# fanxiaochen/Multi-View-Registration

Hardware: NVIDIA B200
Metric: nn_queries_per_s (24-view x 200k turntable registration; ms_per_step = registration ms; a query = one PCL-equivalent nearest-neighbour answer: every source point per iteration + every gated match's reciprocal answer, the oracle's counter) (higher is better)
Workload: dtype f32

## Files before the change

### include/mvr_b200.h

```cpp
#ifndef MVR_B200_H
#define MVR_B200_H

#include <stddef.h>
#include <stdint.h>

#ifdef __cplusplus
extern "C" {
#endif

typedef struct mvr_ctx mvr_ctx;

typedef enum {
  MVR_OK = 0,
  MVR_ERR_BAD_ARG = 1,
  MVR_ERR_TOO_FEW_CORRESPONDENCES = 2,
  MVR_ERR_CUDA = 3,
  MVR_ERR_NO_INPUT = 4,
  MVR_ERR_NOT_SPD = 5,
  MVR_ERR_ALLOC = 6,
  MVR_ERR_NCCL = 7
} mvr_status;

typedef enum { MVR_CLOUD_TARGET = 0, MVR_CLOUD_SOURCE = 1 } mvr_cloud;
typedef enum { MVR_POINT_TO_POINT = 0, MVR_POINT_TO_PLANE = 1, MVR_SYMMETRIC = 2 } mvr_estimator;
typedef enum {
  MVR_REASON_NONE = 0,
  MVR_REASON_ITERATIONS = 1,
  MVR_REASON_TRANSFORM = 2,
  MVR_REASON_ABS_MSE = 3,
  MVR_REASON_REL_MSE = 4,
  MVR_REASON_NO_CORRESPONDENCES = 5
} mvr_reason;

typedef struct {
  int max_iterations;
  double max_correspondence_distance;
  double transformation_epsilon;
  double euclidean_fitness_epsilon;
  int use_reciprocal_correspondences;
  int estimator;
  int fixed_iterations;
  int min_correspondences;
} mvr_icp_params;

typedef struct {
  int iterations;
  int converged;
  int reason;
  int n_correspondences;
  double mse;
  double gpu_ms;
  uint64_t nn_queries;
} mvr_icp_report;

typedef struct {
  int iteration;
  int n_correspondences;
  double mse;
  float delta[16];
} mvr_icp_iteration;

typedef struct {
  float origin[3];
  float inv_cell;
  float cell;
  int bits;
} mvr_grid;

typedef struct {
  uint64_t launches;
  double ms;
  double bytes;
  double units;
} mvr_kernel_stat;

enum { MVR_K_MORTON = 0, MVR_K_SORT = 1, MVR_K_TABLE = 2, MVR_K_NN = 3, MVR_K_CORR = 4, MVR_K_REDUCE = 5,
       MVR_K_TRANSFORM = 6, MVR_K_NORMALS = 7, MVR_K_COUNT = 8 };

const char* mvr_version(void);
uint64_t mvr_kernel_launch_count(void);
void mvr_transfer_sizes(size_t* state_bytes, size_t* log_record_bytes);
const char* mvr_status_string(int status);
void mvr_icp_params_default(mvr_icp_params* p);

int mvr_ctx_create(int device, mvr_ctx** out);
int mvr_ctx_destroy(mvr_ctx* ctx);
int mvr_ctx_set_stream(mvr_ctx* ctx, void* cuda_stream);
int mvr_ctx_synchronize(mvr_ctx* ctx);
void* mvr_ctx_get_stream(mvr_ctx* ctx);
const char* mvr_last_error(mvr_ctx* ctx);
int mvr_ctx_set_profiling(mvr_ctx* ctx, int on);
int mvr_ctx_get_kernel_stats(mvr_ctx* ctx, mvr_kernel_stat* out , int reset);
double mvr_debug_value(mvr_ctx* ctx, int k);
int mvr_ctx_set_index_options(mvr_ctx* ctx, float cell_edge, int max_bits);

int mvr_ctx_set_nn_options(mvr_ctx* ctx, double points_per_cell, double dense_ratio);
typedef enum { MVR_NN_AUTO = 0, MVR_NN_WARP = 1, MVR_NN_THREAD = 2, MVR_NN_CELL = 3, MVR_NN_SEEDED = 4 } mvr_nn_mode;
int mvr_ctx_set_nn_mode(mvr_ctx* ctx, int mode);
int mvr_ctx_set_gate_mask(mvr_ctx* ctx, int on);

int mvr_set_target(mvr_ctx* ctx, const float* xyzw, size_t n);
int mvr_set_source(mvr_ctx* ctx, const float* xyzw, size_t n);
int mvr_set_target_device(mvr_ctx* ctx, const float* d_xyzw, size_t n);
int mvr_set_source_device(mvr_ctx* ctx, const float* d_xyzw, size_t n);
int mvr_set_clouds_device(mvr_ctx* const* ctxs, const int* which, const float* const* d_xyzw, const size_t* n, int count);
int mvr_cloud_share(mvr_ctx* dst, int which_dst , mvr_ctx* src, int which_src);
int mvr_set_target_normals(mvr_ctx* ctx, const float* nxyzc, size_t n);
int mvr_set_source_normals(mvr_ctx* ctx, const float* nxyzc, size_t n);
int mvr_normals_share(mvr_ctx* dst, int which_dst , mvr_ctx* src, int which_src);

int mvr_index_build(mvr_ctx* ctx, int which , const mvr_grid* grid );
int mvr_index_export(mvr_ctx* ctx, int which, mvr_grid* grid, uint32_t* sorted_keys, int32_t* perm,
                     uint32_t* cell_start);

int mvr_nn_query(mvr_ctx* ctx, const float* q_xyzw, size_t n, int32_t* idx, float* d2);
int mvr_nn_query_device(mvr_ctx* ctx, const float* d_q_xyzw, size_t n, int32_t* d_idx, float* d_d2);

int mvr_correspondences(mvr_ctx* ctx, double max_dist, int reciprocal, int32_t* index_query, int32_t* index_match,
                        float* distance, size_t* count);

int mvr_icp_align(mvr_ctx* ctx, const mvr_icp_params* params, const float* guess, float* out_pose, float* out_xyzw,
                  mvr_icp_report* report);
int mvr_icp_align_batch(mvr_ctx* const* ctxs, int count, const mvr_icp_params* params, const float* guesses, float* out_poses,
                        mvr_icp_report* reports, int* statuses);
int mvr_ctx_set_batch_group(mvr_ctx* ctx, int pairs);
int mvr_icp_get_iterations(mvr_ctx* ctx, mvr_icp_iteration* out, int max_records, int* count);
int mvr_fitness_score(mvr_ctx* ctx, double max_range, double* score);

typedef struct {
  double n;
  double origin[3];
  double sa[3], sb[3];
  double sba[9];
  double saa[6], sbb[6];
  double d2;
} mvr_pair_moments;
int mvr_pair_moments_compute(mvr_ctx* ctx, double max_dist, int reciprocal, const float* guess, mvr_pair_moments* out);

int mvr_pair_moments_compute_batch(mvr_ctx* const* ctxs, int count, double max_dist, int reciprocal, const float* guesses,
                                   mvr_pair_moments* out, int* statuses);

int mvr_estimate_normals(mvr_ctx* ctx, int which, int k, const float viewpoint[3], float* out_nxyzc,
                         int32_t* neighbours);
int mvr_estimate_normals_batch(mvr_ctx* const* ctxs, int count, int k, const float* viewpoints, float* const* out_nxyzc,
                               int* statuses);

int mvr_apply_pose(mvr_ctx* ctx, const void* points, size_t n, size_t stride_bytes, const double* pose, float* out_xyzw);
int mvr_apply_pose_device(mvr_ctx* ctx, const void* d_points, size_t n, size_t stride_bytes, const double* pose, float* d_out_xyzw);
int mvr_copy_aligned_device(mvr_ctx* ctx, float* d_out_xyzw);

typedef struct mvr_registrator mvr_registrator;

typedef struct {
  const float* xyzw;
  size_t n;
  int on_device;
  const double* init_pose;
} mvr_view;

typedef enum {
  MVR_REGISTER_RING_PAIRS = 0,
  MVR_REGISTER_ACCUMULATE = 1,
  MVR_REGISTER_ICP = 2,
  MVR_REGISTER_LUM = 3
} mvr_register_mode;

typedef struct {
  double pivot[3];
  double axis[3];
  mvr_icp_params icp;
  int repeat_times;
  int mode;
  int loop_closure;
  int lum_iterations;
  int pair_begin, pair_end;
  int want_fitness;
  int normal_k;
} mvr_turntable_params;

typedef struct {
  int source_view, target_view;
  int status;
  int iterations;
  int n_correspondences;
  double mse;
  double fitness;
  double gpu_ms;
  uint64_t nn_queries;
  float pose[16];
} mvr_pair_report;

typedef struct { int view; int repeat; double score; } mvr_fitness_record;

void mvr_turntable_params_default(mvr_turntable_params* p);
void mvr_turntable_rotation(const double pivot[3], const double axis[3], double angle, double* out16);
double mvr_turntable_view_angle(int view, int n_views);

int mvr_registrator_create(int device, int streams, mvr_registrator** out);
int mvr_registrator_destroy(mvr_registrator* r);
const char* mvr_registrator_last_error(mvr_registrator* r);
mvr_ctx* mvr_registrator_context(mvr_registrator* r, int slot);
int mvr_registrator_streams(mvr_registrator* r);
int mvr_pairwise_align(mvr_registrator* r, const mvr_view* source, const mvr_view* target, const mvr_icp_params* icp,
                       const float* guess, float* out_pose, mvr_icp_report* report);
int mvr_register_turntable(mvr_registrator* r, const mvr_view* views, int n_views, const mvr_turntable_params* prm,
                           float* poses, mvr_pair_report* reports);
typedef struct mvr_multi mvr_multi;
typedef struct {
  float pose[16];
  int32_t n_correspondences, iterations, status, reserved;
  double mse;
  uint64_t nn_queries;
} mvr_pair_record;
int mvr_multi_create(const int* devices, int n_devices, mvr_multi** out);
int mvr_multi_destroy(mvr_multi* m);
const char* mvr_multi_last_error(mvr_multi* m);
int mvr_multi_devices(mvr_multi* m);
int mvr_multi_contexts(mvr_multi* m, int rank);
mvr_ctx* mvr_multi_context(mvr_multi* m, int rank, int slot);
void mvr_multi_pair_range(int rank, int n_ranks, int n_pairs, int* pair_begin, int* pair_end);
int mvr_multi_upload(mvr_multi* m, const mvr_view* views, int n_views);
int mvr_register_turntable_multi(mvr_multi* m, const mvr_view* views, int n_views, const mvr_turntable_params* prm, int use_resident,
                                 float* poses, mvr_pair_report* reports, mvr_pair_record* records, double* device_ms);

int mvr_registrator_get_fitness_log(mvr_registrator* r, mvr_fitness_record* out, int max_records, int* count);
int mvr_compute_error(mvr_registrator* r, const mvr_view* views, int n_views, double max_distance, size_t* counts, double* mean_d2,
                      int* n_pairs);
int mvr_ring_close(const float* rel_poses, const double* weights, int n_views, int relax, int iterations, const double* centre,
                   double rot_scale, float* poses);
int mvr_lum_relax(const mvr_pair_moments* edges, const int* src, const int* tgt, int n_edges, int n_views, int iterations,
                  double* poses);
int mvr_lum_compute(const mvr_pair_moments* edges, const int* src, const int* tgt, int n_edges, int n_views, int iterations,
                    double convergence_threshold, double* poses6, double* transforms);
void mvr_pair_moments_transform(const mvr_pair_moments* in, const double* pose, const double* new_origin, mvr_pair_moments* out);
int mvr_get_bbox(mvr_ctx* ctx, int which, float lo[3], float hi[3]);
int mvr_refine_axis(const float* poses, int count, double pivot[3], double axis[3]);

int mvr_transformation_load(const char* path, double* pose);
int mvr_transformation_save(const char* path, const double* pose);
int mvr_axis_load(const char* path, double pivot[3], double axis[3]);
int mvr_axis_save(const char* path, const double pivot[3], const double axis[3]);
int mvr_points_save_asc(const char* path, const void* rich_points, size_t n);
int mvr_merge_registered(mvr_ctx* ctx, const void* const* views, const size_t* counts, const double* poses, const int* registered,
                         int n_views, int full_matrix_normals, void* out, size_t* out_count);

int mvr_denoise(mvr_ctx* ctx, const void* points, size_t n, size_t stride_bytes, int segment_threshold, double triangle_length,
// ... 7 lines not shown
```

### multi-view-registration_b200/__init__.py

```python
import ctypes as C
import os

import numpy as np

_HERE = os.path.dirname(os.path.abspath(__file__))
LIB_PATH = os.environ.get("MVR_B200_LIB") or os.path.join(_HERE, "libmvr_b200.so")

K_NAMES = ["morton", "sort", "table", "nn", "corr", "reduce", "transform", "normals"]
K_COUNT = 8
(OK, ERR_BAD_ARG, ERR_TOO_FEW, ERR_CUDA, ERR_NO_INPUT, ERR_NOT_SPD, ERR_ALLOC, ERR_NCCL) = range(8)
TARGET, SOURCE = 0, 1
NN_AUTO, NN_WARP, NN_THREAD, NN_CELL, NN_SEEDED = 0, 1, 2, 3, 4
POINT_TO_POINT, POINT_TO_PLANE, SYMMETRIC = 0, 1, 2


class MvrError(RuntimeError):
    def __init__(self, status, msg):
        super().__init__("mvr status %d: %s" % (status, msg))
        self.status = status


class IcpParams(C.Structure):
    _fields_ = [
        ("max_iterations", C.c_int),
        ("max_correspondence_distance", C.c_double),
        ("transformation_epsilon", C.c_double),
        ("euclidean_fitness_epsilon", C.c_double),
        ("use_reciprocal_correspondences", C.c_int),
        ("estimator", C.c_int),
        ("fixed_iterations", C.c_int),
        ("min_correspondences", C.c_int),
    ]


class IcpReport(C.Structure):
    _fields_ = [
        ("iterations", C.c_int),
        ("converged", C.c_int),
        ("reason", C.c_int),
        ("n_correspondences", C.c_int),
        ("mse", C.c_double),
        ("gpu_ms", C.c_double),
        ("nn_queries", C.c_uint64),
    ]


class IcpIteration(C.Structure):
    _fields_ = [("iteration", C.c_int), ("n_correspondences", C.c_int), ("mse", C.c_double), ("delta", C.c_float * 16)]


class Grid(C.Structure):
    _fields_ = [("origin", C.c_float * 3), ("inv_cell", C.c_float), ("cell", C.c_float), ("bits", C.c_int)]


class KernelStat(C.Structure):
    _fields_ = [("launches", C.c_uint64), ("ms", C.c_double), ("bytes", C.c_double), ("units", C.c_double)]


class TurntableParams(C.Structure):
    _fields_ = [
        ("pivot", C.c_double * 3),
        ("axis", C.c_double * 3),
        ("icp", IcpParams),
        ("repeat_times", C.c_int),
        ("mode", C.c_int),
        ("loop_closure", C.c_int),
        ("lum_iterations", C.c_int),
        ("pair_begin", C.c_int),
        ("pair_end", C.c_int),
        ("want_fitness", C.c_int),
        ("normal_k", C.c_int),
    ]


class PairMoments(C.Structure):
    _fields_ = [("n", C.c_double), ("origin", C.c_double * 3), ("sa", C.c_double * 3), ("sb", C.c_double * 3),
                ("sba", C.c_double * 9), ("saa", C.c_double * 6), ("sbb", C.c_double * 6), ("d2", C.c_double)]

    @classmethod
    def from_pairs(cls, a, b, origin=None):
        a = np.asarray(a, dtype=np.float64).reshape(-1, 3)
        b = np.asarray(b, dtype=np.float64).reshape(-1, 3)
        o = np.zeros(3) if origin is None else np.asarray(origin, dtype=np.float64)
        m = cls()
        m.n = float(len(a))
        m.origin[:] = o.tolist()
        if len(a):
            x, y = a - o, b - o
            m.sa[:] = x.sum(0).tolist(); m.sb[:] = y.sum(0).tolist()
            m.sba[:] = (y.T @ x).reshape(9).tolist()
            xx, yy = x.T @ x, y.T @ y
            m.saa[:] = [xx[0, 0], xx[0, 1], xx[0, 2], xx[1, 1], xx[1, 2], xx[2, 2]]
            m.sbb[:] = [yy[0, 0], yy[0, 1], yy[0, 2], yy[1, 1], yy[1, 2], yy[2, 2]]
            m.d2 = float(((a - b) ** 2).sum())
        return m

    def as_dict(self):
        return dict(n=self.n, origin=np.array(self.origin[:]), sa=np.array(self.sa[:]), sb=np.array(self.sb[:]),
                    sba=np.array(self.sba[:]).reshape(3, 3), saa=np.array(self.saa[:]), sbb=np.array(self.sbb[:]), d2=self.d2)


class ViewDesc(C.Structure):
    _fields_ = [("xyzw", C.c_void_p), ("n", C.c_size_t), ("on_device", C.c_int), ("init_pose", C.POINTER(C.c_double))]


class PairRecord(C.Structure):
    _fields_ = [("pose", C.c_float * 16), ("n_correspondences", C.c_int32), ("iterations", C.c_int32), ("status", C.c_int32),
                ("reserved", C.c_int32), ("mse", C.c_double), ("nn_queries", C.c_uint64)]


class FitnessRecord(C.Structure):
    _fields_ = [("view", C.c_int), ("repeat", C.c_int), ("score", C.c_double)]


class PairReport(C.Structure):
    _fields_ = [
        ("source_view", C.c_int),
        ("target_view", C.c_int),
        ("status", C.c_int),
        ("iterations", C.c_int),
        ("n_correspondences", C.c_int),
        ("mse", C.c_double),
        ("fitness", C.c_double),
        ("gpu_ms", C.c_double),
        ("nn_queries", C.c_uint64),
        ("pose", C.c_float * 16),
    ]


REPORT = np.dtype([("source_view", "<i4"), ("target_view", "<i4"), ("status", "<i4"), ("iterations", "<i4"), ("n_correspondences", "<i4"),
                   ("pad", "<i4"), ("mse", "<f8"), ("fitness", "<f8"), ("gpu_ms", "<f8"), ("nn_queries", "<u8"), ("pose", "<f4", (16,))])
assert REPORT.itemsize == C.sizeof(PairReport)


class BoundViews:

    def __init__(self, arr, keep, n, views):
        self.arr, self.keep, self.n, self.views = arr, keep, n, views


RING_PAIRS, ACCUMULATE, ICP_ORDER, LUM = 0, 1, 2, 3

_lib = None


def lib():
    global _lib
    if _lib is not None:
        return _lib
    if not os.path.exists(LIB_PATH):
        raise ImportError("libmvr_b200.so is not built: run `python __graft_entry__.py build` "
                          "(the CUDA library is the only implementation; there is no CPU fallback)")
    L = C.CDLL(LIB_PATH)
    vp, fp, ip, up = C.c_void_p, C.POINTER(C.c_float), C.POINTER(C.c_int32), C.POINTER(C.c_uint32)
    L.mvr_version.restype = C.c_char_p
    L.mvr_kernel_launch_count.restype = C.c_uint64
    L.mvr_status_string.restype = C.c_char_p
    L.mvr_transfer_sizes.argtypes = [C.POINTER(C.c_size_t), C.POINTER(C.c_size_t)]
    L.mvr_transfer_sizes.restype = None
    L.mvr_status_string.argtypes = [C.c_int]
    L.mvr_icp_params_default.argtypes = [C.POINTER(IcpParams)]
    L.mvr_ctx_create.argtypes = [C.c_int, C.POINTER(vp)]
    L.mvr_ctx_destroy.argtypes = [vp]
    L.mvr_ctx_set_stream.argtypes = [vp, vp]
    L.mvr_ctx_synchronize.argtypes = [vp]
    L.mvr_last_error.argtypes = [vp]
    L.mvr_last_error.restype = C.c_char_p
    L.mvr_ctx_set_profiling.argtypes = [vp, C.c_int]
    L.mvr_ctx_get_kernel_stats.argtypes = [vp, C.POINTER(KernelStat), C.c_int]
    L.mvr_debug_value.argtypes = [vp, C.c_int]
    L.mvr_debug_value.restype = C.c_double
    L.mvr_ctx_set_index_options.argtypes = [vp, C.c_float, C.c_int]
    L.mvr_ctx_set_batch_group.argtypes = [vp, C.c_int]
    L.mvr_ctx_set_nn_options.argtypes = [vp, C.c_double, C.c_double]
    L.mvr_ctx_set_nn_mode.argtypes = [vp, C.c_int]
    L.mvr_ctx_set_gate_mask.argtypes = [vp, C.c_int]
    for name in ("mvr_set_target", "mvr_set_source", "mvr_set_target_device", "mvr_set_source_device", "mvr_set_target_normals",
                 "mvr_set_source_normals"):
        getattr(L, name).argtypes = [vp, vp, C.c_size_t]
    L.mvr_normals_share.argtypes = [vp, C.c_int, vp, C.c_int]
    L.mvr_index_build.argtypes = [vp, C.c_int, C.POINTER(Grid)]
    L.mvr_index_export.argtypes = [vp, C.c_int, C.POINTER(Grid), up, ip, up]
    L.mvr_nn_query.argtypes = [vp, fp, C.c_size_t, ip, fp]
    L.mvr_nn_query_device.argtypes = [vp, vp, C.c_size_t, vp, vp]
    L.mvr_correspondences.argtypes = [vp, C.c_double, C.c_int, ip, ip, fp, C.POINTER(C.c_size_t)]
    L.mvr_icp_align.argtypes = [vp, C.POINTER(IcpParams), fp, fp, vp, C.POINTER(IcpReport)]
    L.mvr_icp_align_batch.argtypes = [C.POINTER(vp), C.c_int, C.POINTER(IcpParams), fp, fp, C.POINTER(IcpReport), ip]
    L.mvr_icp_get_iterations.argtypes = [vp, C.POINTER(IcpIteration), C.c_int, C.POINTER(C.c_int)]
    L.mvr_fitness_score.argtypes = [vp, C.c_double, C.POINTER(C.c_double)]
    L.mvr_denoise.argtypes = [vp, vp, C.c_size_t, C.c_size_t, C.c_int, C.c_double, ip, C.POINTER(C.c_size_t), C.POINTER(C.c_size_t)]
    L.mvr_estimate_normals.argtypes = [vp, C.c_int, C.c_int, fp, fp, ip]
    L.mvr_estimate_normals_batch.argtypes = [C.POINTER(vp), C.c_int, C.c_int, fp, C.POINTER(fp), ip]
    dp = C.POINTER(C.c_double)
    L.mvr_apply_pose.argtypes = [vp, vp, C.c_size_t, C.c_size_t, dp, fp]
    L.mvr_apply_pose_device.argtypes = [vp, vp, C.c_size_t, C.c_size_t, dp, vp]
    L.mvr_copy_aligned_device.argtypes = [vp, vp]
    L.mvr_turntable_params_default.argtypes = [C.POINTER(TurntableParams)]
    L.mvr_turntable_rotation.argtypes = [dp, dp, C.c_double, dp]
    L.mvr_turntable_view_angle.argtypes = [C.c_int, C.c_int]
    L.mvr_turntable_view_angle.restype = C.c_double
    L.mvr_registrator_create.argtypes = [C.c_int, C.c_int, C.POINTER(vp)]
    L.mvr_registrator_destroy.argtypes = [vp]
    L.mvr_registrator_last_error.argtypes = [vp]
    L.mvr_registrator_last_error.restype = C.c_char_p
    L.mvr_registrator_context.argtypes = [vp, C.c_int]
    L.mvr_registrator_context.restype = vp
    L.mvr_registrator_streams.argtypes = [vp]
    L.mvr_pairwise_align.argtypes = [vp, C.POINTER(ViewDesc), C.POINTER(ViewDesc), C.POINTER(IcpParams), fp, fp, C.POINTER(IcpReport)]
    L.mvr_register_turntable.argtypes = [vp, C.POINTER(ViewDesc), C.c_int, C.POINTER(TurntableParams), fp, C.POINTER(PairReport)]
    L.mvr_multi_create.argtypes = [ip, C.c_int, C.POINTER(vp)]
    L.mvr_multi_destroy.argtypes = [vp]
    L.mvr_multi_last_error.argtypes = [vp]
    L.mvr_multi_last_error.restype = C.c_char_p
    L.mvr_multi_devices.argtypes = [vp]
    L.mvr_multi_contexts.argtypes = [vp, C.c_int]
    L.mvr_multi_context.argtypes = [vp, C.c_int, C.c_int]
    L.mvr_multi_context.restype = vp
    L.mvr_multi_pair_range.argtypes = [C.c_int, C.c_int, C.c_int, C.POINTER(C.c_int), C.POINTER(C.c_int)]
    L.mvr_multi_pair_range.restype = None
    L.mvr_multi_upload.argtypes = [vp, C.POINTER(ViewDesc), C.c_int]
    L.mvr_register_turntable_multi.argtypes = [vp, C.POINTER(ViewDesc), C.c_int, C.POINTER(TurntableParams), C.c_int, fp, C.POINTER(PairReport),
                                               C.POINTER(PairRecord), dp]
    L.mvr_registrator_get_fitness_log.argtypes = [vp, C.POINTER(FitnessRecord), C.c_int, C.POINTER(C.c_int)]
    L.mvr_compute_error.argtypes = [vp, C.POINTER(ViewDesc), C.c_int, C.c_double, C.POINTER(C.c_size_t), dp, C.POINTER(C.c_int)]
    L.mvr_ring_close.argtypes = [fp, dp, C.c_int, C.c_int, C.c_int, dp, C.c_double, fp]
    L.mvr_get_bbox.argtypes = [vp, C.c_int, fp, fp]
    L.mvr_set_clouds_device.argtypes = [C.POINTER(vp), ip, C.POINTER(vp), C.POINTER(C.c_size_t), C.c_int]
    L.mvr_refine_axis.argtypes = [fp, C.c_int, dp, dp]
    L.mvr_transformation_load.argtypes = [C.c_char_p, dp]
    L.mvr_transformation_save.argtypes = [C.c_char_p, dp]
    L.mvr_axis_load.argtypes = [C.c_char_p, dp, dp]
    L.mvr_axis_save.argtypes = [C.c_char_p, dp, dp]
    L.mvr_points_save_asc.argtypes = [C.c_char_p, vp, C.c_size_t]
    L.mvr_merge_registered.argtypes = [vp, C.POINTER(vp), C.POINTER(C.c_size_t), dp, ip, C.c_int, C.c_int, vp, C.POINTER(C.c_size_t)]
    L.mvr_pair_moments_compute.argtypes = [vp, C.c_double, C.c_int, fp, C.POINTER(PairMoments)]
    L.mvr_lum_relax.argtypes = [C.POINTER(PairMoments), ip, ip, C.c_int, C.c_int, C.c_int, dp]
    L.mvr_lum_compute.argtypes = [C.POINTER(PairMoments), ip, ip, C.c_int, C.c_int, C.c_int, C.c_double, dp, dp]
    L.mvr_pair_moments_transform.argtypes = [C.POINTER(PairMoments), dp, dp, C.POINTER(PairMoments)]
    L.mvr_pair_moments_transform.restype = None
    _lib = L
    return L


def kernel_launch_count():
    return int(lib().mvr_kernel_launch_count())


def _transfer_sizes():
    a, b = C.c_size_t(0), C.c_size_t(0)
    lib().mvr_transfer_sizes(C.byref(a), C.byref(b))
    return int(a.value), int(b.value)


def icp_state_bytes():
    return _transfer_sizes()[0]


def icp_log_record_bytes():
    return _transfer_sizes()[1]


def default_params(**kw):
    p = IcpParams()
    lib().mvr_icp_params_default(C.byref(p))
    alias = {"max_dist": "max_correspondence_distance", "reciprocal": "use_reciprocal_correspondences"}
    for k, v in kw.items():
        setattr(p, alias.get(k, k), v)
    return p


def _pts(a):
    a = np.ascontiguousarray(a, dtype=np.float32)
    if a.ndim != 2 or a.shape[1] != 4:
        raise ValueError("points must be n x 4 float32 (pcl::PointXYZ layout)")
    return a


def _fp(a):
    return a.ctypes.data_as(C.POINTER(C.c_float))


def _ip(a):
    return a.ctypes.data_as(C.POINTER(C.c_int32))


def _up(a):
    return a.ctypes.data_as(C.POINTER(C.c_uint32))


def pose_to_numpy(flat16):
    return np.asarray(flat16, dtype=np.float32).reshape(4, 4).T.copy()


def pose_from_numpy(M):
    return np.ascontiguousarray(np.asarray(M, dtype=np.float32).T).reshape(16)


class Context:

    def __init__(self, device=0, _borrowed=None):
        self._keep = {}
        self._tgt_n = None
        self._owned = _borrowed is None
        if _borrowed is not None:
            self._h = C.c_void_p(_borrowed)
            return
        self._h = C.c_void_p()
        rc = lib().mvr_ctx_create(int(device), C.byref(self._h))
        if rc != OK:
            raise MvrError(rc, "mvr_ctx_create failed (no usable CUDA device %d; there is no CPU fallback)" % device)
        self._keep = {}

    def close(self):
        if getattr(self, "_h", None) and self._h.value:
            if self._owned:
                lib().mvr_ctx_destroy(self._h)
            self._h = C.c_void_p()

    def __del__(self):
        try:
            self.close()
        except Exception:
            pass

    def _ck(self, rc, allow=()):
        if rc != OK and rc not in allow:
            raise MvrError(rc, (lib().mvr_last_error(self._h) or b"").decode() or lib().mvr_status_string(rc).decode())
        return rc

    def set_stream(self, cuda_stream_ptr):
        self._ck(lib().mvr_ctx_set_stream(self._h, C.c_void_p(int(cuda_stream_ptr))))

    def synchronize(self):
        self._ck(lib().mvr_ctx_synchronize(self._h))

    def set_profiling(self, on):
        self._ck(lib().mvr_ctx_set_profiling(self._h, int(bool(on))))

    def kernel_stats(self, reset=False):
        arr = (KernelStat * K_COUNT)()
        self._ck(lib().mvr_ctx_get_kernel_stats(self._h, arr, int(bool(reset))))
        return {K_NAMES[i]: dict(launches=int(arr[i].launches), ms=arr[i].ms, bytes=arr[i].bytes, units=arr[i].units)
                for i in range(K_COUNT)}

    def last_error(self):
        return (lib().mvr_last_error(self._h) or b"").decode()

    def debug_value(self, k):
        return float(lib().mvr_debug_value(self._h, int(k)))

    def set_index_options(self, cell_edge=0.0, max_bits=8):
        self._ck(lib().mvr_ctx_set_index_options(self._h, C.c_float(cell_edge), int(max_bits)))

    def set_nn_options(self, points_per_cell=8.0, dense_ratio=8.0):
        self._ck(lib().mvr_ctx_set_nn_options(self._h, float(points_per_cell), float(dense_ratio)))

    def set_nn_mode(self, mode):
        self._ck(lib().mvr_ctx_set_nn_mode(self._h, int(mode)))

    def set_gate_mask(self, on):
        self._ck(lib().mvr_ctx_set_gate_mask(self._h, 1 if on else 0))

    def set_batch_group(self, pairs):
        self._ck(lib().mvr_ctx_set_batch_group(self._h, int(pairs)))

    def set_target(self, pts):
        pts = _pts(pts)
        self._ck(lib().mvr_set_target(self._h, pts.ctypes.data, len(pts)))
        self._tgt_n = len(pts)

    def set_source(self, pts):
        pts = _pts(pts)
        self._ck(lib().mvr_set_source(self._h, pts.ctypes.data, len(pts)))

    def set_target_device(self, ptr, n, keepalive=None):
        self._keep["tgt"] = keepalive
        self._ck(lib().mvr_set_target_device(self._h, C.c_void_p(int(ptr)), int(n)))
        self._tgt_n = int(n)

    def set_source_device(self, ptr, n, keepalive=None):
        self._keep["src"] = keepalive
        self._ck(lib().mvr_set_source_device(self._h, C.c_void_p(int(ptr)), int(n)))

    def set_target_normals(self, nrm):
        nrm = _pts(nrm)
        self._ck(lib().mvr_set_target_normals(self._h, nrm.ctypes.data, len(nrm)))

    def set_source_normals(self, nrm):
        nrm = _pts(nrm)
        self._ck(lib().mvr_set_source_normals(self._h, nrm.ctypes.data, len(nrm)))

    def normals_share(self, which, other, other_which):
        self._ck(lib().mvr_normals_share(self._h, int(which), other._h, int(other_which)))

    def index_build(self, which=TARGET, grid=None):
        g = None
        if grid is not None:
            g = Grid()
            g.origin[:] = [float(x) for x in grid["origin"]]
            g.inv_cell = float(grid["inv_cell"])
            g.cell = float(grid.get("cell", 1.0 / grid["inv_cell"]))
            g.bits = int(grid["bits"])
        self._ck(lib().mvr_index_build(self._h, int(which), C.byref(g) if g is not None else None))

    def index_export(self, which, n):
        g = Grid()
        self._ck(lib().mvr_index_export(self._h, int(which), C.byref(g), None, None, None))
        keys = np.empty(n, dtype=np.uint32)
        perm = np.empty(n, dtype=np.int32)
        start = np.empty((1 << (3 * g.bits)) + 1, dtype=np.uint32)
        self._ck(lib().mvr_index_export(self._h, int(which), C.byref(g), _up(keys), _ip(perm), _up(start)))
        grid = dict(origin=np.array(g.origin[:], dtype=np.float32), inv_cell=np.float32(g.inv_cell), cell=np.float32(g.cell), bits=g.bits)
        return grid, keys, perm, start

    def nn_query(self, q):
        q = _pts(q)
        idx = np.empty(len(q), dtype=np.int32)
        d2 = np.empty(len(q), dtype=np.float32)
        self._ck(lib().mvr_nn_query(self._h, _fp(q), len(q), _ip(idx), _fp(d2)))
        return idx, d2

    def nn_query_device(self, q_ptr, n, idx_ptr, d2_ptr):
        self._ck(lib().mvr_nn_query_device(self._h, C.c_void_p(int(q_ptr)), int(n), C.c_void_p(int(idx_ptr)), C.c_void_p(int(d2_ptr))))

    def correspondences(self, n_source, max_dist, reciprocal):
        q = np.empty(max(n_source, 1), dtype=np.int32)
        m = np.empty(max(n_source, 1), dtype=np.int32)
        d = np.empty(max(n_source, 1), dtype=np.float32)
        cnt = C.c_size_t(0)
        self._ck(lib().mvr_correspondences(self._h, float(max_dist), int(bool(reciprocal)), _ip(q), _ip(m), _fp(d), C.byref(cnt)))
        c = cnt.value
        return q[:c].copy(), m[:c].copy(), d[:c].copy()

    def icp_align(self, params, guess=None, n_source=None, want_cloud=False):
        g = pose_from_numpy(guess) if guess is not None else None
        fin = np.empty(16, dtype=np.float32)
        cloud = np.empty((n_source, 4), dtype=np.float32) if want_cloud else None
        rep = IcpReport()
        rc = lib().mvr_icp_align(self._h, C.byref(params), _fp(g) if g is not None else None, _fp(fin),
                                 cloud.ctypes.data if cloud is not None else None, C.byref(rep))
        self._ck(rc, allow=(ERR_TOO_FEW, ERR_NOT_SPD))
        cnt = C.c_int(0)
        lib().mvr_icp_get_iterations(self._h, None, 0, C.byref(cnt))
        recs = (IcpIteration * max(cnt.value, 1))()
        lib().mvr_icp_get_iterations(self._h, recs, cnt.value, C.byref(cnt))
        log = [dict(iteration=recs[k].iteration, n_corr=recs[k].n_correspondences, mse=recs[k].mse,
                    delta=pose_to_numpy(recs[k].delta[:])) for k in range(cnt.value)]
        return dict(status=rc, final=pose_to_numpy(fin), cloud=cloud, iterations=rep.iterations, converged=rep.converged,
                    reason=rep.reason, n_corr=rep.n_correspondences, mse=rep.mse, gpu_ms=rep.gpu_ms,
                    nn_queries=int(rep.nn_queries), log=log)

    def pair_moments(self, max_dist, reciprocal=True, guess=None):
        g = pose_from_numpy(guess) if guess is not None else None
        m = PairMoments()
        self._ck(lib().mvr_pair_moments_compute(self._h, float(max_dist), int(bool(reciprocal)), _fp(g) if g is not None else None, C.byref(m)))
        return m

    def merge_registered(self, views, poses, registered=None, full_matrix_normals=True):
        arrs = [np.ascontiguousarray(v, dtype=RICH_POINT) for v in views]
        V = len(arrs)
        ptrs = (C.c_void_p * max(V, 1))(*[a.ctypes.data for a in arrs])
        counts = (C.c_size_t * max(V, 1))(*[len(a) for a in arrs])
        P = np.ascontiguousarray(np.stack([np.asarray(T, dtype=np.float64).T.reshape(16) for T in poses])) if V else np.zeros((1, 16))
        reg = None if registered is None else np.ascontiguousarray(registered, dtype=np.int32)
        total = C.c_size_t(0)
        self._ck(lib().mvr_merge_registered(self._h, ptrs, counts, _dp(P), _ip(reg) if reg is not None else None, V, int(bool(full_matrix_normals)), None, C.byref(total)))
        out = np.empty(total.value, dtype=RICH_POINT)
        if total.value:
            self._ck(lib().mvr_merge_registered(self._h, ptrs, counts, _dp(P), _ip(reg) if reg is not None else None, V, int(bool(full_matrix_normals)),
                                                out.ctypes.data, C.byref(total)))
        return out

    def iterations(self):
        cnt = C.c_int(0)
        self._ck(lib().mvr_icp_get_iterations(self._h, None, 0, C.byref(cnt)))
        recs = (IcpIteration * max(cnt.value, 1))()
        self._ck(lib().mvr_icp_get_iterations(self._h, recs, cnt.value, C.byref(cnt)))
        return [dict(iteration=recs[k].iteration, n_corr=recs[k].n_correspondences, mse=recs[k].mse,
                     delta=pose_to_numpy(recs[k].delta[:])) for k in range(cnt.value)]

    def fitness_score(self, max_range=None):
        import sys
        s = C.c_double(0)
        self._ck(lib().mvr_fitness_score(self._h, sys.float_info.max if max_range is None else float(max_range), C.byref(s)))
        return s.value

    def estimate_normals(self, which, n, k, viewpoint=(0.0, 0.0, 0.0), want_neighbours=False):
        vp = np.ascontiguousarray(viewpoint, dtype=np.float32)
        out = np.empty((n, 4), dtype=np.float32)
        nbr = np.empty((n, k), dtype=np.int32) if want_neighbours else None
        self._ck(lib().mvr_estimate_normals(self._h, int(which), int(k), _fp(vp), _fp(out), _ip(nbr) if nbr is not None else None))
        return (out, nbr) if want_neighbours else out


    def denoise(self, pts, segment_threshold=10, triangle_length=2.5):
        a = np.ascontiguousarray(pts)
        n = len(a)
        stride = a.dtype.itemsize if a.dtype.fields else a.strides[0]
        keep = np.empty(max(n, 1), dtype=np.int32)
        cnt, noise = C.c_size_t(0), C.c_size_t(0)
        self._ck(lib().mvr_denoise(self._h, a.ctypes.data, n, stride, int(segment_threshold), float(triangle_length), _ip(keep), C.byref(cnt), C.byref(noise)))
        return keep[:cnt.value].copy(), int(noise.value)

# ... 347 lines not shown
```

### multi-view-registration_b200/build.py

```python
import os
import shutil
import subprocess
import sys

HERE = os.path.dirname(os.path.abspath(__file__))
CSRC = os.path.join(HERE, "csrc")
HOST = os.path.join(HERE, "host")
LIB = os.path.join(HERE, "libmvr_b200.so")

CU_SOURCES = ["index.cu", "bin.cu", "pair_index.cu", "cell_nn.cu", "icp.cu", "normals.cu", "denoise.cu", "api.cu"]
HOST_SOURCES = ["registrator.cpp", "lum.cpp", "capi.cpp", "multi.cpp"]

NVCC_FLAGS = [
    "-O3", "-std=c++17",
    "-gencode", "arch=compute_100a,code=sm_100a",
    "-lineinfo",
    "-Xcompiler", "-fPIC",
    "-fmad=false",
    "-Xcompiler", "-fno-fast-math",
]


def _nvcc():
    for cand in (os.environ.get("NVCC"), shutil.which("nvcc"), "/usr/local/cuda/bin/nvcc"):
        if cand and os.path.exists(cand):
            return cand
    raise RuntimeError("nvcc not found: the CUDA path cannot be built (there is no CPU fallback)")


def sources():
    srcs = [os.path.join(CSRC, f) for f in CU_SOURCES]
    srcs += [os.path.join(HOST, f) for f in HOST_SOURCES if os.path.exists(os.path.join(HOST, f))]
    return srcs


def deps():
    out = []
    for d in (CSRC, HOST, os.path.join(os.path.dirname(HERE), "include")):
        if os.path.isdir(d):
            out += [os.path.join(d, f) for f in os.listdir(d)]
    return out


def stale():
    if not os.path.exists(LIB):
        return True
    t = os.path.getmtime(LIB)
    return any(os.path.getmtime(p) > t for p in deps())


def build(force=False, verbose=False, out=None):
    if out is None and not force and not stale():
        return LIB
    extra = os.environ.get("MVR_NVCC_DEFS", "").split()
    cmd = [_nvcc()] + NVCC_FLAGS + extra + ["-shared", "-o", out or LIB, "-x", "cu"] + sources() + ["-ldl"]
    if verbose:
        cmd += ["-Xptxas", "-v"]
        print(" ".join(cmd))
    env = dict(os.environ)
    res = subprocess.run(cmd, stdout=subprocess.PIPE, stderr=subprocess.STDOUT, text=True, env=env)
    if verbose or res.returncode != 0:
        sys.stderr.write(res.stdout)
    if res.returncode != 0:
        raise RuntimeError("nvcc failed building libmvr_b200.so")
    return out or LIB


if __name__ == "__main__":
    print(build(force="--force" in sys.argv, verbose="-v" in sys.argv))
```

### multi-view-registration_b200/csrc/api.cu

```cuda
#include <cfloat>
#include <chrono>
#include <cstdlib>
#include <climits>
#include <cmath>
#include <cstdio>
#include <cstring>
#include <memory>
#include <string>
#include <thread>
#include <vector>

#include "../../include/mvr_b200.h"
#include "launch.h"
#include "small_solve.h"

#ifndef MVR_PG_XRATIO
#define MVR_PG_XRATIO 4
#endif

using namespace mvr;

#include <atomic>
namespace mvr {
static std::atomic<unsigned long long> g_launches{0};
void count_launch(int n) { g_launches.fetch_add((unsigned long long)n, std::memory_order_relaxed); }
unsigned long long launch_count() { return g_launches.load(std::memory_order_relaxed); }
int estimate_normals_batch(mvr_ctx* const* ctxs, const int* which, int count, int k, const float* viewpoints, float* const* out_nxyzc,
                           int* statuses);
}

namespace {

struct DevBuf {
  void* p = nullptr;
  size_t cap = 0;
  cudaError_t ensure(size_t bytes) {
    if (bytes <= cap) return cudaSuccess;
    if (p) cudaFree(p);
    p = nullptr; cap = 0;
    size_t want = bytes + bytes / 8 + 256;
    cudaError_t e = cudaMalloc(&p, want);
    if (e == cudaSuccess) cap = want;
    return e;
  }
  void release() { if (p) cudaFree(p); p = nullptr; cap = 0; }
  template <class T> T* as() const { return (T*)p; }
};

struct Cloud {
  const float4* pts = nullptr;
  DevBuf own;
  int n = 0;
  float lo[3] = {0, 0, 0}, hi[3] = {0, 0, 0};
  int n_bad = 0;
  uint64_t gen = 0;
  bool index_valid = false;
  bool exportable = false;
  uint64_t index_gen = 0;
  mvr_grid grid{};
  GridDev gd{};
  DevBuf keys, vals, keys_alt, vals_alt, hist, counters, sorted, table;
  uint32_t* sorted_keys = nullptr;
  uint32_t* perm = nullptr;
  IndexDev dev() const {
    IndexDev ix;
    ix.pts = sorted.as<float4>(); ix.start = table.as<uint32_t>(); ix.g = gd; ix.n_valid = n - n_bad;
    return ix;
  }
  void release() {
    own.release(); keys.release(); vals.release(); keys_alt.release(); vals_alt.release(); hist.release();
    counters.release(); sorted.release(); table.release();
  }
};

struct ProfRec { int kind; cudaEvent_t a, b; double bytes, units; int count; };

struct PairIndex {
  DevBuf sorted, start, s0;
  DevBuf gocc, gmask;
  float gm_gate = -1.f;
  int gm_stride = 0;
  PairGrid g{};
  uint32_t cells = 0;
  int n_valid = 0;
  uint64_t gen = 0;
  bool valid = false;
  void release() { sorted.release(); start.release(); s0.release(); gocc.release(); gmask.release(); gm_gate = -1.f; valid = false; }
};

}

struct mvr_ctx {
  int device = 0;
  cudaStream_t stream = nullptr;
  bool own_stream = false;
  Cloud tgt, src;
  DevBuf normals, snormals;
  const float4* tnrm = nullptr;
  const float4* snrm = nullptr;
  DevBuf nsrc;
  Mat4f guess_m{};
  DevBuf cur, corr_p, corr_j, corr_d2, rmin, rnn, partials, sums, out_cloud, qtmp, itmp, ftmp, scratch, misc, tiles, state, log;
  PairIndex pt, ps;
  PairIndex nt, nq;
  double nn_ppc = 8.0;
  double nn_dense_ratio = 8.0;
  int nn_mode = MVR_NN_AUTO;
  int nn_sorted_from = 262144;
  bool gate_mask = false;
  FwdArgs fa{}; RevArgs ra{};
  bool want_rnn = false;
  int group_pairs = 0;
  struct BuildScratch { DevBuf keys, vals, moved, count, tiles; uint32_t epoch = 1; } bs[2];
  DevBuf stage_dev;
  IcpState* h_stage = nullptr;
  int stage_cap = 0;
  DevBuf bbox_dev;
  uint32_t* h_bbox = nullptr;
  int log_pending = 0;
  bool out_pending = false;
  DevBuf crowded;
  uint32_t crowded_seen = 0;
  IcpState* h_state = nullptr;
  IterRec* h_log = nullptr;
  double* h_sums = nullptr;
  uint32_t* h_small = nullptr;
  std::string err;
  bool profiling = false;
  std::vector<ProfRec> prof;
  std::vector<cudaEvent_t> ev_pool;
  mvr_kernel_stat stats[MVR_K_COUNT] = {};
  std::vector<mvr_icp_iteration> iters;
  bool have_out = false;
  float cell_edge_opt = 0.f;
  int max_bits_opt = 8;
  cudaEvent_t ev_a = nullptr, ev_b = nullptr;
};

namespace {

#define CK(expr)                                                                                 \
  do {                                                                                           \
    cudaError_t _e = (expr);                                                                     \
    if (_e != cudaSuccess) {                                                                     \
      ctx->err = std::string(#expr) + ": " + cudaGetErrorString(_e);                             \
      return MVR_ERR_CUDA;                                                                       \
    }                                                                                            \
  } while (0)

int fail(mvr_ctx* ctx, int code, const char* msg) {
  if (ctx) ctx->err = msg;
  return code;
}

cudaEvent_t get_event(mvr_ctx* ctx) {
  if (!ctx->ev_pool.empty()) { cudaEvent_t e = ctx->ev_pool.back(); ctx->ev_pool.pop_back(); return e; }
  cudaEvent_t e = nullptr;
  cudaEventCreate(&e);
  return e;
}

struct ProfScope {
  mvr_ctx* ctx; int idx;
  cudaStream_t st;
  ProfScope(mvr_ctx* c, int kind, double bytes, double units, int count = 1, cudaStream_t stream = nullptr) : ctx(c), idx(-1), st(stream ? stream : c->stream) {
    if (!c->profiling) return;
    ProfRec r{kind, get_event(c), get_event(c), bytes, units, count};
    cudaEventRecord(r.a, st);
    c->prof.push_back(r);
    idx = (int)c->prof.size() - 1;
  }
  ~ProfScope() { if (idx >= 0) cudaEventRecord(ctx->prof[idx].b, st); }
};

void prof_flush(mvr_ctx* ctx) {
  for (ProfRec& r : ctx->prof) {
    cudaEventSynchronize(r.b);
    float ms = 0.f;
    if (cudaEventElapsedTime(&ms, r.a, r.b) == cudaSuccess) {
      mvr_kernel_stat& s = ctx->stats[r.kind];
      s.launches += (uint64_t)r.count; s.ms += ms; s.bytes += r.bytes; s.units += r.units;
    }
    ctx->ev_pool.push_back(r.a); ctx->ev_pool.push_back(r.b);
  }
  ctx->prof.clear();
}

double density_cell_edge(const float lo[3], const float hi[3], int n, double ppc) {
  double ex = std::max(0.0, (double)hi[0] - lo[0]), ey = std::max(0.0, (double)hi[1] - lo[1]), ez = std::max(0.0, (double)hi[2] - lo[2]);
  double area = ex * ey + ey * ez + ex * ez;
  double ext = std::max(ex, std::max(ey, ez));
  if (n <= 0 || ext <= 0) return 1.0;
  if (area <= 0) return ext / std::min(1024.0, std::max(1.0, (double)n / ppc));
  return std::sqrt(1.5 * ppc * area / (double)n);
}

mvr_grid make_grid(const float lo[3], const float hi[3], double cell, int max_bits) {
  mvr_grid g{};
  double ext = 0;
  for (int a = 0; a < 3; ++a) ext = std::max(ext, (double)hi[a] - (double)lo[a]);
  if (!(ext > 0) || !std::isfinite(ext)) ext = 1.0;
  if (!(cell > 0) || !std::isfinite(cell)) cell = ext;
  if (max_bits > 10) max_bits = 10;
  if (max_bits < 1) max_bits = 1;
  int bits = std::min(3, max_bits);
  while (bits < max_bits && cell * (double)(1 << bits) < ext * 1.0001) ++bits;
  if (cell * (double)(1 << bits) < ext * 1.0001) cell = ext * 1.0001 / (double)(1 << bits);
  for (int a = 0; a < 3; ++a) g.origin[a] = lo[a];
  g.inv_cell = (float)(1.0 / cell);
  g.cell = (float)cell;
  g.bits = bits;
  return g;
}

GridDev to_dev(const mvr_grid& g) {
  GridDev d;
  d.ox = g.origin[0]; d.oy = g.origin[1]; d.oz = g.origin[2];
  d.inv_cell = g.inv_cell;
  double c = (1.0 / (double)g.inv_cell) * (1.0 - 1e-6);
  d.cell_lo = std::nextafterf((float)c, 0.0f);
  d.bits = g.bits;
  d.G = 1 << g.bits;
  return d;
}

bool same_grid(const mvr_grid& a, const mvr_grid& b) {
  return std::memcmp(a.origin, b.origin, sizeof(a.origin)) == 0 && a.inv_cell == b.inv_cell && a.bits == b.bits;
}

int cloud_bbox(mvr_ctx* ctx, Cloud& c) {
  for (int a = 0; a < 3; ++a) { c.lo[a] = 0; c.hi[a] = 0; }
  c.n_bad = 0;
  if (c.n <= 0) return MVR_OK;
  CK(ctx->misc.ensure(64));
  uint32_t* d = ctx->misc.as<uint32_t>();
  CK(launch_bbox_init(d, ctx->stream));
  CK(launch_bbox(c.pts, c.n, d, ctx->stream));
  CK(cudaMemcpyAsync(ctx->h_small, d, 7 * sizeof(uint32_t), cudaMemcpyDeviceToHost, ctx->stream));
  CK(cudaStreamSynchronize(ctx->stream));
  c.n_bad = (int)ctx->h_small[6];
  if (c.n_bad < c.n)
    for (int a = 0; a < 3; ++a) { c.lo[a] = bbox_decode(ctx->h_small[a]); c.hi[a] = bbox_decode(ctx->h_small[3 + a]); }
  return MVR_OK;
}

int cloud_set(mvr_ctx* ctx, Cloud& c, const float* xyzw, size_t n, bool device_ptr) {
  if (n > (size_t)INT_MAX / 2) return fail(ctx, MVR_ERR_BAD_ARG, "cloud too large");
  if (n > 0 && !xyzw) return fail(ctx, MVR_ERR_BAD_ARG, "null point pointer");
  c.index_valid = false;
  c.gen++;
  c.n = (int)n;
  if (device_ptr) {
    c.pts = (const float4*)xyzw;
  } else {
    CK(c.own.ensure(std::max<size_t>(n, 1) * sizeof(float4)));
    if (n) CK(cudaMemcpyAsync(c.own.p, xyzw, n * sizeof(float4), cudaMemcpyHostToDevice, ctx->stream));
    c.pts = c.own.as<float4>();
  }
  return cloud_bbox(ctx, c);
}

int build_index(mvr_ctx* ctx, Cloud& c, const float4* pts, const mvr_grid& g) {
  const int n = c.n;
  const size_t cells = (size_t)1 << (3 * g.bits);
  CK(c.keys.ensure(std::max(n, 1) * sizeof(uint32_t)));
  CK(c.vals.ensure(std::max(n, 1) * sizeof(uint32_t)));
  CK(c.keys_alt.ensure(std::max(n, 1) * sizeof(uint32_t)));
  CK(c.vals_alt.ensure(std::max(n, 1) * sizeof(uint32_t)));
  CK(c.hist.ensure((size_t)256 * radix_num_blocks(n) * sizeof(uint32_t)));
  CK(c.sorted.ensure(std::max(n, 1) * sizeof(float4)));
  CK(c.table.ensure((cells + 2) * sizeof(uint32_t)));
  c.grid = g;
  c.gd = to_dev(g);
  {
    ProfScope ps(ctx, MVR_K_MORTON, 24.0 * n, n);
    CK(launch_morton_keys(pts, n, c.gd, c.keys.as<uint32_t>(), c.vals.as<uint32_t>(), ctx->stream));
  }
  int key_bits = 3 * g.bits + (c.n_bad > 0 ? 1 : 0);
  SortScratch sc{c.keys_alt.as<uint32_t>(), c.vals_alt.as<uint32_t>(), c.hist.as<uint32_t>()};
  {
    ProfScope ps(ctx, MVR_K_SORT, 16.0 * n, n);
    CK(launch_radix_sort(c.keys.as<uint32_t>(), c.vals.as<uint32_t>(), n, key_bits, sc, &c.sorted_keys, &c.perm, ctx->stream));
  }
  {
    ProfScope ps(ctx, MVR_K_TABLE, 36.0 * n + 4.0 * (double)cells, n);
    CK(launch_gather_sorted(pts, c.perm, n, c.sorted.as<float4>(), ctx->stream));
    CK(launch_cell_table(c.sorted_keys, n, g.bits, c.table.as<uint32_t>(), ctx->stream));
  }
  c.index_valid = true;
  c.exportable = true;
  c.index_gen = c.gen;
  return MVR_OK;
}

mvr_grid auto_grid(mvr_ctx* ctx, const Cloud& c) {
  double e = ctx->cell_edge_opt > 0 ? ctx->cell_edge_opt : density_cell_edge(c.lo, c.hi, c.n - c.n_bad, 6.0);
  return make_grid(c.lo, c.hi, e, ctx->max_bits_opt);
}

PairGrid make_pair_grid(const float lo[3], const float hi[3], double e, uint32_t* cells_out, int xr = 1);
bool same_pair_grid(const PairGrid& a, const PairGrid& b);
int build_pair_index(mvr_ctx* ctx, PairIndex& ix, const float4* pts, int n, int n_bad, const Mat4f* guess, const PairGrid& g,
                     uint32_t cells, bool keep_s0, bool ordered = true);
int plan_pair_index(mvr_ctx* ctx, PairIndex& ix, int slot, const float4* pts, int n, int n_bad, const Mat4f* guess, const PairGrid& g,
                    uint32_t cells, bool ordered, cudaStream_t stream, BuildJob* job);
int run_pair_builds(mvr_ctx* ctx, const BuildJob* jobs, int count, cudaStream_t stream);

double pair_cell_edge(mvr_ctx* ctx, const Cloud& c, double max_dist);

int nn_pass_dense(mvr_ctx* ctx, const float4* q, int n, int32_t* d_idx, float* d_d2, bool seeded) {
  Cloud& t = ctx->tgt;
  const int mv = t.n - t.n_bad;
  const double e = ctx->cell_edge_opt > 0 ? ctx->cell_edge_opt : density_cell_edge(t.lo, t.hi, mv, ctx->nn_ppc);
  uint32_t cells = 0;
  const PairGrid g = make_pair_grid(t.lo, t.hi, e, &cells);
  int rc;
  if (!(ctx->nt.valid && ctx->nt.gen == t.gen && same_pair_grid(ctx->nt.g, g))) {
    if ((rc = build_pair_index(ctx, ctx->nt, t.pts, t.n, t.n_bad, nullptr, g, cells, false))) return rc;
    ctx->nt.gen = t.gen;
  }
  if ((rc = build_pair_index(ctx, ctx->nq, q, n, 0, nullptr, g, cells, false, false))) return rc;
  ProfScope ps(ctx, MVR_K_NN, 24.0 * n + 16.0 * t.n, (double)n);
  if (seeded)
    CK(launch_seeded_nn(ctx->nq.sorted.as<float4>(), n, ctx->nq.start.as<uint32_t>() + cells, ctx->nt.sorted.as<float4>(),
                        ctx->nt.start.as<uint32_t>(), g, mv, d_idx, d_d2, ctx->stream));
  else
    CK(launch_cell_nn(ctx->nq.sorted.as<float4>(), n, ctx->nq.start.as<uint32_t>() + cells, ctx->nt.sorted.as<float4>(),
                      ctx->nt.start.as<uint32_t>(), g, mv, d_idx, d_d2, ctx->stream));
  return MVR_OK;
}

int nn_pass(mvr_ctx* ctx, const float4* q, int n, int32_t* d_idx, float* d_d2) {
  if (ctx->nn_mode == MVR_NN_CELL) return nn_pass_dense(ctx, q, n, d_idx, d_d2, false);
  if (ctx->nn_mode == MVR_NN_SEEDED || (ctx->nn_mode == MVR_NN_AUTO && n > ctx->nn_sorted_from)) return nn_pass_dense(ctx, q, n, d_idx, d_d2, true);
  Cloud& t = ctx->tgt;
  PairIndex& pt = ctx->pt;
  int rc;
  if (!(pt.valid && pt.gen == t.gen && pt.g.xr == 1.0f)) {
    uint32_t cells = 0;
    const PairGrid gt = make_pair_grid(t.lo, t.hi, pair_cell_edge(ctx, t, INFINITY), &cells);
    if ((rc = build_pair_index(ctx, pt, t.pts, t.n, t.n_bad, nullptr, gt, cells, false))) return rc;
    pt.gen = t.gen;
  }
  ProfScope ps(ctx, MVR_K_NN, 24.0 * n + 16.0 * t.n, (double)n);
  if (ctx->nn_mode == MVR_NN_WARP || (ctx->nn_mode == MVR_NN_AUTO && n <= 131072)) {
    CK(launch_warp_nn(q, n, pt.sorted.as<float4>(), pt.start.as<uint32_t>(), pt.g, pt.n_valid, d_idx, d_d2, ctx->stream));
    return MVR_OK;
  }
  const bool sorted = n > 262144;
  if (sorted && (rc = build_pair_index(ctx, ctx->nq, q, n, 0, nullptr, pt.g, pt.cells, false, false))) return rc;
  CK(launch_pair_nn(sorted ? ctx->nq.sorted.as<float4>() : q, n, sorted, pt.sorted.as<float4>(), pt.start.as<uint32_t>(), pt.g, pt.n_valid, d_idx,
                    d_d2, ctx->stream));
  return MVR_OK;
}

void mat_identity(float* m) { for (int k = 0; k < 16; ++k) m[k] = (k % 5 == 0) ? 1.f : 0.f; }

float gate_float(double max_dist) {
  double m2 = max_dist * max_dist;
  if (!(m2 < (double)FLT_MAX)) return INFINITY;
  float f = (float)m2;
  if ((double)f < m2) f = std::nextafterf(f, INFINITY);
  return std::nextafterf(f, INFINITY);
}

double pair_cell_edge(mvr_ctx* ctx, const Cloud& c, double max_dist) {
  if (ctx->cell_edge_opt > 0) return ctx->cell_edge_opt;
  const int nv = c.n - c.n_bad;
  const double e_lo = density_cell_edge(c.lo, c.hi, nv, 2.0), e_hi = density_cell_edge(c.lo, c.hi, nv, 12.0);
  const double m2 = max_dist * max_dist;
  return (m2 < 1e30) ? std::min(std::max(0.5 * max_dist * 1.002, e_lo), e_hi) : density_cell_edge(c.lo, c.hi, nv, 6.0);
}

PairGrid make_pair_grid(const float lo[3], const float hi[3], double e, uint32_t* cells_out, int xr) {
  const double max_cells = 16.0 * 1024 * 1024;
  if (xr != 1 && xr != 2 && xr != 4 && xr != 8) xr = 1;
  double ext[3];
  for (int a = 0; a < 3; ++a) {
    ext[a] = (double)hi[a] - (double)lo[a];
    if (!(ext[a] >= 0) || !std::isfinite(ext[a])) ext[a] = 0;
  }
  if (!(e > 0) || !std::isfinite(e)) e = std::max(1e-3, std::max(ext[0], std::max(ext[1], ext[2])));
  int n[3];
  for (;;) {
    double tot = 1;
    for (int a = 0; a < 3; ++a) {
      const int r = a == 0 ? xr : 1;
      n[a] = (int)std::min(4096.0 * r, std::floor(ext[a] / (e / r)) + 3.0 * r);
      tot *= n[a];
    }
    if (tot <= max_cells) break;
    if (xr > 1) { xr /= 2; continue; }
    e *= 1.25;
  }
  PairGrid g;
  g.ox = lo[0] - (float)e; g.oy = lo[1] - (float)e; g.oz = lo[2] - (float)e;
  if (!std::isfinite(g.ox)) g.ox = 0.f;
  if (!std::isfinite(g.oy)) g.oy = 0.f;
  if (!std::isfinite(g.oz)) g.oz = 0.f;
  g.inv_cell = (float)(1.0 / e);
  g.cell_lo = std::nextafterf((float)((1.0 / (double)g.inv_cell) * (1.0 - 1e-6)), 0.0f);
  g.nx = n[0]; g.ny = n[1]; g.nz = n[2];
  g.xr = (float)xr;
  g.inv_cell_x = g.inv_cell * g.xr;
  *cells_out = (uint32_t)n[0] * (uint32_t)n[1] * (uint32_t)n[2];
  return g;
}

bool same_pair_grid(const PairGrid& a, const PairGrid& b) { return std::memcmp(&a, &b, sizeof(PairGrid)) == 0; }

int plan_pair_index(mvr_ctx* ctx, PairIndex& ix, int slot, const float4* pts, int n, int n_bad, const Mat4f* guess, const PairGrid& g,
                    uint32_t cells, bool ordered, cudaStream_t stream, BuildJob* job) {
  mvr_ctx::BuildScratch& bs = ctx->bs[slot];
  const size_t nn = (size_t)std::max(n, 1);
  CK(bs.keys.ensure(nn * sizeof(uint32_t)));
  CK(bs.vals.ensure(nn * sizeof(uint32_t)));
  if (ordered) CK(bs.moved.ensure(nn * sizeof(float4)));
  CK(ix.sorted.ensure(nn * sizeof(float4)));
  CK(ix.start.ensure(((size_t)cells + 2) * sizeof(uint32_t)));
  if (((size_t)cells + 1) * sizeof(uint32_t) > bs.count.cap) {
    CK(bs.count.ensure(((size_t)cells + 1) * sizeof(uint32_t)));
    CK(cudaMemsetAsync(bs.count.p, 0, bs.count.cap, stream));
  }
  const int ntiles = scan_num_tiles((size_t)cells + 1);
  const size_t tiles = (size_t)ntiles + 1;
  if (tiles * sizeof(unsigned long long) > bs.tiles.cap) {
    CK(bs.tiles.ensure(tiles * sizeof(unsigned long long)));
    CK(cudaMemsetAsync(bs.tiles.p, 0, bs.tiles.cap, stream));
  }
  if (!ctx->crowded.p) { CK(ctx->crowded.ensure(64)); CK(cudaMemsetAsync(ctx->crowded.p, 0, 64, stream)); }
  BuildJob& j = *job;
  j = BuildJob{};
  j.in = pts; j.n = n; j.apply = guess ? 1 : 0;
  if (guess) j.M = *guess;
  j.g = g; j.cells = cells;
  j.keys = bs.keys.as<uint32_t>(); j.rank = bs.vals.as<uint32_t>(); j.counters = bs.count.as<uint32_t>();
  j.tiles = bs.tiles.as<unsigned long long>(); j.epoch = bs.epoch; j.ntiles = ntiles;
  bs.epoch = (bs.epoch % 0x3fffffffu) + 1;
  j.tmp = ordered ? bs.moved.as<float4>() : nullptr; j.sorted = ix.sorted.as<float4>(); j.start = ix.start.as<uint32_t>();
  j.crowded = ctx->crowded.as<uint32_t>(); j.ordered = ordered ? 1 : 0;
  ix.g = g; ix.cells = cells; ix.n_valid = n - n_bad; ix.valid = true; ix.gm_gate = -1.f;
  return MVR_OK;
}

int run_pair_builds(mvr_ctx* ctx, const BuildJob* jobs, int count, cudaStream_t stream) {
  for (int k0 = 0; k0 < count; k0 += BUILD_MAX_JOBS) {
    const int c = std::min(count - k0, (int)BUILD_MAX_JOBS);
    BuildBatch batch;
    double bytes = 0, pts = 0;
    for (int k = 0; k < c; ++k) { batch.j[k] = jobs[k0 + k]; bytes += 32.0 * jobs[k0 + k].n + 8.0 * jobs[k0 + k].cells; pts += jobs[k0 + k].n; }
    ProfScope ps(ctx, MVR_K_SORT, bytes, pts, 1, stream);
    CK(launch_pair_builds(batch, c, stream));
  }
  return MVR_OK;
}

int build_pair_index(mvr_ctx* ctx, PairIndex& ix, const float4* pts, int n, int n_bad, const Mat4f* guess, const PairGrid& g,
                     uint32_t cells, bool keep_s0, bool ordered) {
  (void)keep_s0;
  BuildJob job;
  ix.valid = false;
  int rc = plan_pair_index(ctx, ix, &ix == &ctx->pt || &ix == &ctx->nt ? 0 : 1, pts, n, n_bad, guess, g, cells, ordered, ctx->stream, &job);
  if (rc) { ix.valid = false; return rc; }
  return run_pair_builds(ctx, &job, 1, ctx->stream);
}

int ensure_gate_mask(mvr_ctx* ctx, PairIndex& ix, float max_d2f, cudaStream_t stream) {
  if (!ctx->gate_mask || !(max_d2f < 3.0e38f) || ix.n_valid <= 0) { ix.gm_gate = -1.f; return MVR_OK; }
  if (ix.gm_gate == max_d2f) return MVR_OK;
  const double slack = 2.0 * ((double)MVR_CELL_MARGIN + 1.0e-6 * (double)std::max(ix.g.nx, std::max(ix.g.ny, ix.g.nz)));
  const double need = std::sqrt((double)max_d2f) * (1.0 + 1.0e-5) / (double)ix.g.cell_lo + slack;
  const int D = (int)std::ceil(need);
  const int Dx = (int)std::ceil(need * (double)ix.g.xr);
  ix.gm_gate = -1.f;
  if (D < 1 || D > 6 || Dx > 31) return MVR_OK;
  const int wstride = (ix.g.nx + 31) / 32;
  const size_t words = (size_t)ix.g.ny * ix.g.nz * wstride;
  CK(ix.gocc.ensure(words * sizeof(uint32_t)));
  CK(ix.gmask.ensure(words * sizeof(uint32_t)));
  CK(launch_gate_mask(ix.start.as<uint32_t>(), ix.g, wstride, D, Dx, ix.gocc.as<uint32_t>(), ix.gmask.as<uint32_t>(), stream));
  ix.gm_stride = wstride;
  ix.gm_gate = max_d2f;
  return MVR_OK;
}

int ensure_pinned(mvr_ctx* ctx) {
  if (!ctx->h_sums) CK(cudaMallocHost((void**)&ctx->h_sums, REDUCE_MAX_VALS * sizeof(double)));
  if (!ctx->h_small) CK(cudaMallocHost((void**)&ctx->h_small, 64 * sizeof(uint32_t)));
  if (!ctx->h_state) CK(cudaMallocHost((void**)&ctx->h_state, sizeof(IcpState)));
  if (!ctx->h_log) CK(cudaMallocHost((void**)&ctx->h_log, ICP_MAX_LOG * sizeof(IterRec)));
  return MVR_OK;
}

template <class F>
void parallel_for(int n, F fn) {
  static const int max_threads = [] { const char* e = std::getenv("MVR_HOST_THREADS"); const int v = e ? std::atoi(e) : 6; return v < 1 ? 1 : (v > 64 ? 64 : v); }();
  const int nt = std::min(max_threads, n);
  if (nt <= 1) { for (int k = 0; k < n; ++k) fn(k); return; }
  std::atomic<int> next{0};
  auto work = [&] { for (int k = next.fetch_add(1); k < n; k = next.fetch_add(1)) fn(k); };
  std::vector<std::thread> th;
  for (int t = 1; t < nt; ++t) th.emplace_back(work);
  work();
  for (std::thread& t : th) t.join();
}

PairGrid normals_grid(const mvr_ctx* ctx, const Cloud& c, int k, uint32_t* cells) {
  const double e = ctx->cell_edge_opt > 0 ? ctx->cell_edge_opt : density_cell_edge(c.lo, c.hi, c.n - c.n_bad, std::max(2.0, k / 3.0));
  return make_pair_grid(c.lo, c.hi, e, cells);
}

NormalsJob normals_job(const PairIndex& ix, int n, const float* viewpoint, float4* out, int32_t* nbr) {
  NormalsJob j{};
  j.sorted = ix.sorted.as<float4>(); j.start = ix.start.as<uint32_t>(); j.g = ix.g;
  j.n = n; j.n_valid = ix.n_valid;
  j.viewpoint = viewpoint ? make_float3(viewpoint[0], viewpoint[1], viewpoint[2]) : make_float3(0.f, 0.f, 0.f);
  j.out = out; j.nbr = nbr;
  return j;
}


}

extern "C" {

const char* mvr_version(void) { return "mvr_b200 0.1 (sm_100a)"; }

uint64_t mvr_kernel_launch_count(void) { return (uint64_t)launch_count(); }

void mvr_transfer_sizes(size_t* state_bytes, size_t* log_record_bytes) {
  if (state_bytes) *state_bytes = sizeof(IcpState);
  if (log_record_bytes) *log_record_bytes = sizeof(IterRec);
}

const char* mvr_status_string(int s) {
  switch (s) {
    case MVR_OK: return "ok";
    case MVR_ERR_BAD_ARG: return "bad argument";
    case MVR_ERR_TOO_FEW_CORRESPONDENCES: return "not enough correspondences";
    case MVR_ERR_CUDA: return "CUDA error";
    case MVR_ERR_NO_INPUT: return "input cloud not set";
    case MVR_ERR_NOT_SPD: return "normal equations not positive definite";
    case MVR_ERR_ALLOC: return "allocation failed";
    case MVR_ERR_NCCL: return "NCCL unavailable or a collective failed";
    default: return "unknown status";
  }
}

void mvr_icp_params_default(mvr_icp_params* p) {
  if (!p) return;
  p->max_iterations = 10;
  p->max_correspondence_distance = std::sqrt(DBL_MAX);
  p->transformation_epsilon = 0.0;
  p->euclidean_fitness_epsilon = -DBL_MAX;
  p->use_reciprocal_correspondences = 0;
  p->estimator = MVR_POINT_TO_POINT;
  p->fixed_iterations = 0;
  p->min_correspondences = 3;
}

int mvr_ctx_create(int device, mvr_ctx** out) {
  if (!out) return MVR_ERR_BAD_ARG;
  *out = nullptr;
  int count = 0;
  if (cudaGetDeviceCount(&count) != cudaSuccess || count <= 0 || device < 0 || device >= count) return MVR_ERR_CUDA;
  if (cudaSetDevice(device) != cudaSuccess) return MVR_ERR_CUDA;
  mvr_ctx* ctx = new mvr_ctx();
  ctx->device = device;
  if (cudaStreamCreateWithFlags(&ctx->stream, cudaStreamNonBlocking) != cudaSuccess) { delete ctx; return MVR_ERR_CUDA; }
  ctx->own_stream = true;
  cudaEventCreate(&ctx->ev_a);
  cudaEventCreate(&ctx->ev_b);
  if (ensure_pinned(ctx) != MVR_OK) { mvr_ctx_destroy(ctx); return MVR_ERR_CUDA; }
  *out = ctx;
  return MVR_OK;
}

int mvr_ctx_destroy(mvr_ctx* ctx) {
  if (!ctx) return MVR_OK;
  cudaSetDevice(ctx->device);
  cudaStreamSynchronize(ctx->stream);
  prof_flush(ctx);
  for (cudaEvent_t e : ctx->ev_pool) cudaEventDestroy(e);
  if (ctx->ev_a) cudaEventDestroy(ctx->ev_a);
  if (ctx->ev_b) cudaEventDestroy(ctx->ev_b);
  ctx->tgt.release(); ctx->src.release(); ctx->normals.release(); ctx->snormals.release(); ctx->nsrc.release();
  ctx->pt.release(); ctx->ps.release(); ctx->nt.release(); ctx->nq.release();
  for (auto& b : ctx->bs) { b.keys.release(); b.vals.release(); b.moved.release(); b.count.release(); b.tiles.release(); }
  ctx->stage_dev.release(); ctx->bbox_dev.release();
  if (ctx->h_stage) cudaFreeHost(ctx->h_stage);
  if (ctx->h_bbox) cudaFreeHost(ctx->h_bbox);
  DevBuf* bufs[] = {&ctx->cur, &ctx->corr_p, &ctx->rmin, &ctx->rnn, &ctx->corr_j, &ctx->corr_d2, &ctx->partials, &ctx->sums, &ctx->out_cloud, &ctx->qtmp,
                    &ctx->itmp, &ctx->ftmp, &ctx->scratch, &ctx->misc, &ctx->tiles, &ctx->state, &ctx->log, &ctx->crowded};
  for (DevBuf* b : bufs) b->release();
  if (ctx->h_sums) cudaFreeHost(ctx->h_sums);
  if (ctx->h_small) cudaFreeHost(ctx->h_small);
  if (ctx->h_state) cudaFreeHost(ctx->h_state);
  if (ctx->h_log) cudaFreeHost(ctx->h_log);
  if (ctx->own_stream && ctx->stream) cudaStreamDestroy(ctx->stream);
  delete ctx;
  return MVR_OK;
}

int mvr_ctx_set_stream(mvr_ctx* ctx, void* s) {
  if (!ctx) return MVR_ERR_BAD_ARG;
  cudaSetDevice(ctx->device);
  cudaStreamSynchronize(ctx->stream);
  if (ctx->own_stream && ctx->stream) cudaStreamDestroy(ctx->stream);
  ctx->stream = (cudaStream_t)s;
  ctx->own_stream = false;
  return MVR_OK;
}

void* mvr_ctx_get_stream(mvr_ctx* ctx) { return ctx ? (void*)ctx->stream : nullptr; }

int mvr_ctx_synchronize(mvr_ctx* ctx) {
  if (!ctx) return MVR_ERR_BAD_ARG;
  CK(cudaStreamSynchronize(ctx->stream));
  return MVR_OK;
}

const char* mvr_last_error(mvr_ctx* ctx) { return ctx ? ctx->err.c_str() : "null context"; }

int mvr_ctx_set_profiling(mvr_ctx* ctx, int on) {
  if (!ctx) return MVR_ERR_BAD_ARG;
  ctx->profiling = on != 0;
  return MVR_OK;
}

int mvr_ctx_get_kernel_stats(mvr_ctx* ctx, mvr_kernel_stat* out, int reset) {
  if (!ctx || !out) return MVR_ERR_BAD_ARG;
  cudaSetDevice(ctx->device);
  CK(cudaStreamSynchronize(ctx->stream));
  prof_flush(ctx);
  std::memcpy(out, ctx->stats, sizeof(ctx->stats));
  if (reset) std::memset(ctx->stats, 0, sizeof(ctx->stats));
  return MVR_OK;
}

int mvr_ctx_set_index_options(mvr_ctx* ctx, float cell_edge, int max_bits) {
  if (!ctx) return MVR_ERR_BAD_ARG;
  if (max_bits < 1 || max_bits > 10) return fail(ctx, MVR_ERR_BAD_ARG, "max_bits must be in 1..10");
  ctx->cell_edge_opt = cell_edge > 0 ? cell_edge : 0.f;
  ctx->max_bits_opt = max_bits;
  ctx->tgt.index_valid = false;
  ctx->src.index_valid = false;
  return MVR_OK;
}

int mvr_ctx_set_nn_options(mvr_ctx* ctx, double points_per_cell, double dense_ratio) {
  if (!ctx || !(points_per_cell > 0) || !(dense_ratio >= 0)) return MVR_ERR_BAD_ARG;
  ctx->nn_ppc = points_per_cell;
  ctx->nn_dense_ratio = dense_ratio;
  ctx->nt.valid = false;
  return MVR_OK;
}

int mvr_ctx_set_gate_mask(mvr_ctx* ctx, int on) {
  if (!ctx) return MVR_ERR_BAD_ARG;
  ctx->gate_mask = on != 0;
  ctx->pt.gm_gate = -1.f;
  return MVR_OK;
}

int mvr_ctx_set_nn_mode(mvr_ctx* ctx, int mode) {
  if (!ctx || mode < MVR_NN_AUTO || mode > MVR_NN_SEEDED) return MVR_ERR_BAD_ARG;
  ctx->nn_mode = mode;
  return MVR_OK;
}

int mvr_ctx_set_batch_group(mvr_ctx* ctx, int pairs) {
  if (!ctx || pairs < 0 || pairs > (int)FUSED_MAX_PAIRS) return MVR_ERR_BAD_ARG;
  ctx->group_pairs = pairs;
  return MVR_OK;
}

int mvr_set_target(mvr_ctx* ctx, const float* xyzw, size_t n) {
  if (!ctx) return MVR_ERR_BAD_ARG;
  cudaSetDevice(ctx->device);
  ctx->tnrm = nullptr;
  return cloud_set(ctx, ctx->tgt, xyzw, n, false);
}
int mvr_set_source(mvr_ctx* ctx, const float* xyzw, size_t n) {
  if (!ctx) return MVR_ERR_BAD_ARG;
  cudaSetDevice(ctx->device);
  ctx->have_out = false;
  ctx->snrm = nullptr;
  return cloud_set(ctx, ctx->src, xyzw, n, false);
}
int mvr_set_target_device(mvr_ctx* ctx, const float* d, size_t n) {
  if (!ctx) return MVR_ERR_BAD_ARG;
  cudaSetDevice(ctx->device);
  ctx->tnrm = nullptr;
  return cloud_set(ctx, ctx->tgt, d, n, true);
}
int mvr_set_source_device(mvr_ctx* ctx, const float* d, size_t n) {
  if (!ctx) return MVR_ERR_BAD_ARG;
  cudaSetDevice(ctx->device);
  ctx->have_out = false;
  ctx->snrm = nullptr;
  return cloud_set(ctx, ctx->src, d, n, true);
}

int mvr_set_clouds_device(mvr_ctx* const* ctxs, const int* which, const float* const* d_xyzw, const size_t* n, int count) {
  if (count < 0 || (count && (!ctxs || !which || !d_xyzw || !n))) return MVR_ERR_BAD_ARG;
  if (count == 0) return MVR_OK;
  mvr_ctx* ctx = ctxs[0];
  if (!ctx) return MVR_ERR_BAD_ARG;
  for (int k = 0; k < count; ++k) {
    if (!ctxs[k] || (which[k] != MVR_CLOUD_TARGET && which[k] != MVR_CLOUD_SOURCE)) return MVR_ERR_BAD_ARG;
    if (ctxs[k]->device != ctx->device) return fail(ctx, MVR_ERR_BAD_ARG, "the contexts of a batch must share a device");
    if (n[k] > (size_t)INT_MAX / 2) return fail(ctx, MVR_ERR_BAD_ARG, "cloud too large");
    if (n[k] > 0 && !d_xyzw[k]) return fail(ctx, MVR_ERR_BAD_ARG, "null point pointer");
  }
  cudaSetDevice(ctx->device);
  if (!ctx->h_bbox) CK(cudaMallocHost((void**)&ctx->h_bbox, (size_t)BBOX_MAX_JOBS * 7 * sizeof(uint32_t)));
  CK(ctx->bbox_dev.ensure((size_t)BBOX_MAX_JOBS * 7 * sizeof(uint32_t)));
  for (int k0 = 0; k0 < count; k0 += BBOX_MAX_JOBS) {
    const int c = std::min(count - k0, (int)BBOX_MAX_JOBS);
    BboxBatch bb;
    for (int k = 0; k < c; ++k) { bb.j[k].pts = (const float4*)d_xyzw[k0 + k]; bb.j[k].n = (int)n[k0 + k]; bb.j[k].pad_ = 0; }
    CK(launch_bbox_batch(bb, c, ctx->bbox_dev.as<uint32_t>(), ctx->stream));
    CK(cudaMemcpyAsync(ctx->h_bbox, ctx->bbox_dev.p, (size_t)c * 7 * sizeof(uint32_t), cudaMemcpyDeviceToHost, ctx->stream));
    CK(cudaStreamSynchronize(ctx->stream));
    for (int k = 0; k < c; ++k) {
      mvr_ctx* m = ctxs[k0 + k];
      Cloud& cl = which[k0 + k] == MVR_CLOUD_TARGET ? m->tgt : m->src;
      if (which[k0 + k] == MVR_CLOUD_TARGET) m->tnrm = nullptr; else { m->have_out = false; m->out_pending = false; m->snrm = nullptr; }
      cl.index_valid = false;
      cl.gen++;
      cl.n = (int)n[k0 + k];
      cl.pts = (const float4*)d_xyzw[k0 + k];
      const uint32_t* w = ctx->h_bbox + 7 * k;
      for (int a = 0; a < 3; ++a) { cl.lo[a] = 0; cl.hi[a] = 0; }
      cl.n_bad = cl.n > 0 ? (int)w[6] : 0;
      if (cl.n > 0 && cl.n_bad < cl.n)
        for (int a = 0; a < 3; ++a) { cl.lo[a] = bbox_decode(w[a]); cl.hi[a] = bbox_decode(w[3 + a]); }
    }
  }
  return MVR_OK;
}
// ... 364 lines not shown
  cudaSetDevice(ctx->device);
  const bool reciprocal = prm->use_reciprocal_correspondences != 0;
  const int gsz = batch_group_size(ctx, count);
  struct Group {
    int g0, gn, gf, gr, enqueued, first, todo;
    bool done, fetched;
    long long n_tot, m_tot;
    mvr_ctx* lead;
    FwdBatch fb;
    RevBatch rb;
  };
  long long batch_points = 0;
  for (int k = 0; k < count; ++k) batch_points += ctxs[k]->fa.n_valid;
  static const int fwd_items_env = [] { const char* e = std::getenv("MVR_FWD_ITEMS"); return e ? std::atoi(e) : 0; }();
  const int fwd_items = fwd_items_env > 0 ? fwd_items_env : (int)std::min<long long>(4, std::max<long long>(1, (batch_points + 300000) / 600000));
  std::vector<Group> groups;
  for (int g0 = 0; g0 < count; g0 += gsz) {
    Group g{};
    g.g0 = g0; g.gn = std::min(gsz, count - g0); g.gf = 1; g.gr = 1; g.enqueued = 0; g.first = 1; g.done = true; g.fetched = true;
    g.lead = ctxs[g0];
    for (int k = 0; k < g.gn; ++k) {
      mvr_ctx* c = ctxs[g0 + k];
      g.fb.a[k] = c->fa; g.rb.a[k] = c->ra;
      if (reciprocal && fwd_items > 1) g.fb.a[k].grid = std::max(1, (c->fa.n_valid + FUSED_THREADS * fwd_items - 1) / (FUSED_THREADS * fwd_items));
      g.gf = std::max(g.gf, g.fb.a[k].grid); g.gr = std::max(g.gr, c->ra.grid);
      if (!c->h_state->done) g.done = false;
      g.n_tot += c->src.n; g.m_tot += c->tgt.n;
    }
    groups.push_back(g);
  }
  int rc0 = ensure_stage(ctx, count);
  if (rc0) return rc0;
  if (ctx->profiling) {
    for (Group& g : groups) CK(cudaStreamSynchronize(g.lead->stream));
    CK(cudaEventRecord(ctx->ev_a, ctx->stream));
    for (size_t gi = 1; gi < groups.size(); ++gi) CK(cudaStreamWaitEvent(groups[gi].lead->stream, ctx->ev_a, 0));
  } else {
    CK(cudaEventRecord(ctx->ev_a, ctx->stream));
  }
  auto unpack = [&](Group& g) {
    if (g.fetched) return;
    g.fetched = true;
    for (int k = 0; k < g.gn; ++k) {
      mvr_ctx* c = ctxs[g.g0 + k];
      std::memcpy(c->h_state, ctx->h_stage + g.g0 + k, sizeof(IcpState));
      c->crowded_seen = std::max(c->crowded_seen, (uint32_t)c->h_state->dbg[3]);
      c->h_state->dbg[3] = 0;
    }
  };
  for (int k = 0; k < count; ++k) ctxs[k]->crowded_seen = 0;
  int batch = prm->fixed_iterations ? 64 : 2;
  for (;;) {
    bool any = false;
    int todo_max = 0;
    std::vector<std::unique_ptr<ProfScope>> scopes;
    for (Group& g : groups) {
      g.todo = 0;
      if (g.done) continue;
      any = true;
      g.todo = std::min(batch, std::max(prm->max_iterations - g.enqueued, 1));
      todo_max = std::max(todo_max, g.todo);
      const double per_it = 16.0 * g.n_tot + 16.0 * g.m_tot + (reciprocal ? 52.0 * g.n_tot : 0.0);
      scopes.emplace_back(new ProfScope(g.lead, MVR_K_CORR, per_it * g.todo, (double)g.n_tot * g.todo, g.todo));
    }
    for (int it = 0; it < todo_max; ++it)
      for (Group& g : groups) {
        if (it >= g.todo) continue;
        CK(launch_icp_forward(g.fb, g.gn, g.gf, g.first, reciprocal, est, g.lead->stream));
        g.first = 0;
        if (reciprocal) CK(launch_icp_reverse(g.rb, g.gn, g.gr, est, g.lead->stream));
      }
    scopes.clear();
    for (Group& g : groups) {
      if (g.todo == 0) continue;
      g.enqueued += g.todo;
      for (int k0 = 0; k0 < g.gn; k0 += BUILD_MAX_JOBS) {
        const int c = std::min(g.gn - k0, (int)BUILD_MAX_JOBS);
        InitBatch ib;
        for (int k = 0; k < c; ++k) ib.j[k] = init_job_of(ctxs[g.g0 + k0 + k]);
        IcpState* d = ctx->stage_dev.as<IcpState>() + g.g0 + k0;
        CK(launch_align_gather(ib, c, d, g.lead->stream));
        CK(cudaMemcpyAsync(ctx->h_stage + g.g0 + k0, d, (size_t)c * sizeof(IcpState), cudaMemcpyDeviceToHost, g.lead->stream));
      }
      g.fetched = false;
    }
    if (!any) break;
    bool more = false;
    for (Group& g : groups) {
      if (g.done) continue;
      if (prm->fixed_iterations) {
        g.done = g.enqueued >= prm->max_iterations;
      } else {
        CK(cudaStreamSynchronize(g.lead->stream));
        unpack(g);
        g.done = true;
        for (int k = 0; k < g.gn; ++k) if (!ctxs[g.g0 + k]->h_state->done) g.done = false;
      }
      if (!g.done) more = true;
    }
    if (!more) break;
    batch = std::min(batch * 2, 64);
  }
  for (size_t gi = 1; gi < groups.size(); ++gi) {
    CK(cudaEventRecord(groups[gi].lead->ev_a, groups[gi].lead->stream));
    CK(cudaStreamWaitEvent(ctx->stream, groups[gi].lead->ev_a, 0));
  }
  CK(cudaEventRecord(ctx->ev_b, ctx->stream));
  CK(cudaStreamSynchronize(ctx->stream));
  for (Group& g : groups) unpack(g);
  return MVR_OK;
}

static int materialize_out(mvr_ctx* ctx) {
  if (!ctx->have_out || !ctx->out_pending) return MVR_OK;
  const int n = ctx->src.n;
  CK(ctx->out_cloud.ensure((size_t)std::max(n, 1) * sizeof(float4)));
  {
    ProfScope ps(ctx, MVR_K_TRANSFORM, 32.0 * n, n);
    CK(launch_transform_final(ctx->src.pts, ctx->out_cloud.as<float4>(), n, ctx->state.as<IcpState>(), ctx->stream));
  }
  ctx->out_pending = false;
  return MVR_OK;
}

static int fetch_log(mvr_ctx* ctx) {
  const int n_log = ctx->log_pending;
  if (n_log <= 0) return MVR_OK;
  ctx->log_pending = 0;
  CK(cudaMemcpyAsync(ctx->h_log, ctx->log.p, (size_t)n_log * sizeof(IterRec), cudaMemcpyDeviceToHost, ctx->stream));
  CK(cudaStreamSynchronize(ctx->stream));
  for (int k = 0; k < n_log; ++k) {
    mvr_icp_iteration rec;
    rec.iteration = ctx->h_log[k].iteration; rec.n_correspondences = ctx->h_log[k].n_corr; rec.mse = ctx->h_log[k].mse;
    std::memcpy(rec.delta, ctx->h_log[k].delta, sizeof(rec.delta));
    ctx->iters.push_back(rec);
  }
  return MVR_OK;
}

static int align_finish_collect(mvr_ctx* ctx, mvr_ctx* lead, float* out_pose, mvr_icp_report* report, int batch_pairs = 1) {
  const IcpState& h = *ctx->h_state;
  if (h.dbg[2] != 0) return fail(ctx, MVR_ERR_CUDA, "internal error: a reciprocal search lost its chooser (search bound violated)");
  ctx->have_out = true; ctx->out_pending = true;
  ctx->log_pending = std::min(h.iter, (int)ICP_MAX_LOG);
  if (out_pose) for (int k = 0; k < 16; ++k) out_pose[k] = (float)h.fin[k];
  if (report) {
    float ms = 0.f;
    cudaEventElapsedTime(&ms, lead->ev_a, lead->ev_b);
    report->iterations = h.iter; report->converged = (h.done && h.status == 0) ? 1 : 0; report->reason = h.reason;
    report->n_correspondences = h.n_corr; report->mse = h.cur_mse; report->nn_queries = h.queries;
    report->gpu_ms = (double)ms / (double)std::max(batch_pairs, 1);
  }
  if (ctx->crowded_seen)
    ctx->err = "warning: a grid cell holds " + std::to_string(ctx->crowded_seen) + " points (duplicates or clamped outliers?): index build and search slow down, sums over it lose their fixed order";
  if (h.status == MVR_ERR_TOO_FEW_CORRESPONDENCES) ctx->err = "not enough correspondences";
  if (h.status == MVR_ERR_NOT_SPD) ctx->err = h.p2l == 2 ? "symmetric point-to-plane normal equations not positive definite" : "point-to-plane normal equations not positive definite";
  return h.status;
}

static int align_finish(mvr_ctx* ctx, mvr_ctx* lead, float* out_pose, float* out_xyzw, mvr_icp_report* report) {
  const int status = align_finish_collect(ctx, lead, out_pose, report);
  if (out_xyzw && ctx->have_out) {
    int rc = materialize_out(ctx);
    if (rc) return rc;
    CK(cudaMemcpyAsync(out_xyzw, ctx->out_cloud.p, (size_t)ctx->src.n * sizeof(float4), cudaMemcpyDeviceToHost, ctx->stream));
    CK(cudaStreamSynchronize(ctx->stream));
  }
  return status;
}

static int icp_align_impl(mvr_ctx* ctx, const mvr_icp_params* prm, const float* guess, float* out_pose, float* out_xyzw,
                          mvr_icp_report* report, bool moments) {
  if (!ctx || !prm) return MVR_ERR_BAD_ARG;
  const int est = estimator_code(prm->estimator);
  if (moments && est != EST_P2P) return fail(ctx, MVR_ERR_BAD_ARG, "pair moments are point-to-point statistics");
  const int est_run = moments ? EST_MOM : est;
  int rc = align_prepare(ctx, prm, guess, est_run);
  if (rc) return rc;
  if ((rc = align_run(&ctx, 1, prm, est_run))) return rc;
  return align_finish(ctx, ctx, out_pose, out_xyzw, report);
}

int mvr_icp_align(mvr_ctx* ctx, const mvr_icp_params* prm, const float* guess, float* out_pose, float* out_xyzw,
                  mvr_icp_report* report) {
  return icp_align_impl(ctx, prm, guess, out_pose, out_xyzw, report, false);
}

int mvr_icp_align_batch(mvr_ctx* const* ctxs, int count, const mvr_icp_params* prm, const float* guesses, float* out_poses,
                        mvr_icp_report* reports, int* statuses) {
  if (count < 0 || (count && (!ctxs || !statuses)) || !prm) return MVR_ERR_BAD_ARG;
  if (count == 0) return MVR_OK;
  for (int k = 0; k < count; ++k) {
    if (!ctxs[k]) return MVR_ERR_BAD_ARG;
    for (int j = 0; j < k; ++j) if (ctxs[j] == ctxs[k]) return fail(ctxs[0], MVR_ERR_BAD_ARG, "a context appears twice in the batch");
    if (ctxs[k]->device != ctxs[0]->device) return fail(ctxs[0], MVR_ERR_BAD_ARG, "the contexts of a batch must share a device");
  }
  const int est = estimator_code(prm->estimator);
  std::vector<mvr_ctx*> ok;
  std::vector<int> slot;
  const bool timing = std::getenv("MVR_DEBUG_TIMING") != nullptr;
  auto now = [] { return std::chrono::duration<double, std::milli>(std::chrono::steady_clock::now().time_since_epoch()).count(); };
  const double t0 = now();
  int rc = align_prepare_batch(ctxs, count, prm, guesses, est, statuses, ok, slot);
  if (rc) { if (!ok.empty() && ok[0] != ctxs[0]) ctxs[0]->err = ok[0]->err; return rc; }
  if (ok.empty()) return MVR_OK;
  const double t1 = now();
  rc = align_run(ok.data(), (int)ok.size(), prm, est);
  if (timing) std::fprintf(stderr, "[timing]   prepare (host enqueue) %.3f ms, run %.3f ms\n", t1 - t0, now() - t1);
  if (rc) { if (ok[0] != ctxs[0]) ctxs[0]->err = ok[0]->err; return rc; }
  for (size_t j = 0; j < ok.size(); ++j) {
    const int k = slot[j];
    statuses[k] = align_finish_collect(ok[j], ok[0], out_poses ? out_poses + 16 * k : nullptr, reports ? reports + k : nullptr, (int)ok.size());
  }
  return MVR_OK;
}

int mvr_pair_moments_compute(mvr_ctx* ctx, double max_dist, int reciprocal, const float* guess, mvr_pair_moments* out) {
  if (!ctx || !out) return MVR_ERR_BAD_ARG;
  std::memset(out, 0, sizeof(*out));
  mvr_icp_params one;
  mvr_icp_params_default(&one);
  one.max_iterations = 1; one.fixed_iterations = 1;
  one.use_reciprocal_correspondences = reciprocal ? 1 : 0;
  one.max_correspondence_distance = max_dist;
  one.min_correspondences = 1;
  mvr_icp_report rep{};
  const int rc = icp_align_impl(ctx, &one, guess, nullptr, nullptr, &rep, true);
  if (rc != MVR_OK && rc != MVR_ERR_TOO_FEW_CORRESPONDENCES) return rc;
  const IcpState& h = *ctx->h_state;
  out->origin[0] = h.ox; out->origin[1] = h.oy; out->origin[2] = h.oz;
  if (rc == MVR_OK) {
    out->n = h.sums[0];
    for (int k = 0; k < 3; ++k) { out->sa[k] = h.sums[1 + k]; out->sb[k] = h.sums[4 + k]; }
    for (int k = 0; k < 9; ++k) out->sba[k] = h.sums[7 + k];
    out->d2 = h.sums[16];
    for (int k = 0; k < 6; ++k) { out->saa[k] = h.sums[17 + k]; out->sbb[k] = h.sums[23 + k]; }
  }
  return MVR_OK;
}

static void moments_from_state(const IcpState& h, bool have, mvr_pair_moments* out) {
  std::memset(out, 0, sizeof(*out));
  out->origin[0] = h.ox; out->origin[1] = h.oy; out->origin[2] = h.oz;
  if (!have) return;
  out->n = h.sums[0];
  for (int k = 0; k < 3; ++k) { out->sa[k] = h.sums[1 + k]; out->sb[k] = h.sums[4 + k]; }
  for (int k = 0; k < 9; ++k) out->sba[k] = h.sums[7 + k];
  out->d2 = h.sums[16];
  for (int k = 0; k < 6; ++k) { out->saa[k] = h.sums[17 + k]; out->sbb[k] = h.sums[23 + k]; }
}

int mvr_pair_moments_compute_batch(mvr_ctx* const* ctxs, int count, double max_dist, int reciprocal, const float* guesses,
                                   mvr_pair_moments* out, int* statuses) {
  if (count < 0 || (count && (!ctxs || !out || !statuses))) return MVR_ERR_BAD_ARG;
  if (count == 0) return MVR_OK;
  for (int k = 0; k < count; ++k) {
    if (!ctxs[k]) return MVR_ERR_BAD_ARG;
    for (int j = 0; j < k; ++j) if (ctxs[j] == ctxs[k]) return fail(ctxs[0], MVR_ERR_BAD_ARG, "a context appears twice in the batch");
    if (ctxs[k]->device != ctxs[0]->device) return fail(ctxs[0], MVR_ERR_BAD_ARG, "the contexts of a batch must share a device");
  }
  mvr_icp_params one;
  mvr_icp_params_default(&one);
  one.max_iterations = 1; one.fixed_iterations = 1;
  one.use_reciprocal_correspondences = reciprocal ? 1 : 0;
  one.max_correspondence_distance = max_dist;
  one.min_correspondences = 1;
  std::vector<mvr_ctx*> ok;
  std::vector<int> slot;
  for (int k = 0; k < count; ++k) std::memset(out + k, 0, sizeof(mvr_pair_moments));
  int rc = align_prepare_batch(ctxs, count, &one, guesses, EST_MOM, statuses, ok, slot);
  if (rc) { if (!ok.empty() && ok[0] != ctxs[0]) ctxs[0]->err = ok[0]->err; return rc; }
  if (ok.empty()) return MVR_OK;
  rc = align_run(ok.data(), (int)ok.size(), &one, EST_MOM);
  if (rc) { if (ok[0] != ctxs[0]) ctxs[0]->err = ok[0]->err; return rc; }
  for (size_t j = 0; j < ok.size(); ++j) {
    const IcpState& h = *ok[j]->h_state;
    const int k = slot[j];
    if (h.dbg[2] != 0) { statuses[k] = fail(ok[j], MVR_ERR_CUDA, "internal error: a reciprocal search lost its chooser (search bound violated)"); continue; }
    const bool have = h.status == MVR_OK;
    statuses[k] = (have || h.status == MVR_ERR_TOO_FEW_CORRESPONDENCES) ? MVR_OK : h.status;
    moments_from_state(h, have, out + k);
    ok[j]->have_out = false; ok[j]->out_pending = false;
  }
  return MVR_OK;
}

double mvr_debug_value(mvr_ctx* ctx, int k) {
  if (ctx && k == 8) return (double)ctx->crowded_seen;
  if (!ctx || !ctx->h_state || k < 0 || k >= 8) return 0.0;
  return (double)ctx->h_state->dbg[k];
}

int mvr_icp_get_iterations(mvr_ctx* ctx, mvr_icp_iteration* out, int max_records, int* count) {
  if (!ctx || !count) return MVR_ERR_BAD_ARG;
  cudaSetDevice(ctx->device);
  int rcl = fetch_log(ctx);
  if (rcl) return rcl;
  int c = (int)ctx->iters.size();
  if (out) {
    int m = std::min(c, std::max(max_records, 0));
    if (m) std::memcpy(out, ctx->iters.data(), (size_t)m * sizeof(mvr_icp_iteration));
    *count = m;
  } else {
    *count = c;
  }
  return MVR_OK;
}

int mvr_fitness_score(mvr_ctx* ctx, double max_range, double* score) {
  if (!ctx || !score) return MVR_ERR_BAD_ARG;
  cudaSetDevice(ctx->device);
  if (ctx->tgt.gen == 0 || ctx->src.gen == 0) return fail(ctx, MVR_ERR_NO_INPUT, "source/target not set");
  const int n = ctx->src.n;
  *score = DBL_MAX;
  if (n == 0 || ctx->tgt.n == 0) return MVR_OK;
  int rc = materialize_out(ctx);
  if (rc) return rc;
  const float4* cloud = ctx->have_out ? ctx->out_cloud.as<float4>() : ctx->src.pts;
  CK(ctx->itmp.ensure((size_t)n * sizeof(int32_t)));
  CK(ctx->ftmp.ensure((size_t)n * sizeof(float)));
  CK(ctx->partials.ensure((size_t)REDUCE_BLOCKS * REDUCE_MAX_VALS * sizeof(double)));
  CK(ctx->sums.ensure(REDUCE_MAX_VALS * sizeof(double)));
  if ((rc = nn_pass(ctx, cloud, n, ctx->itmp.as<int32_t>(), ctx->ftmp.as<float>()))) return rc;
  CK(launch_reduce_fitness(ctx->itmp.as<int32_t>(), ctx->ftmp.as<float>(), n, max_range, ctx->partials.as<double>(),
                           ctx->sums.as<double>(), ctx->stream));
  CK(cudaMemcpyAsync(ctx->h_sums, ctx->sums.p, 2 * sizeof(double), cudaMemcpyDeviceToHost, ctx->stream));
  CK(cudaStreamSynchronize(ctx->stream));
  if (ctx->h_sums[1] > 0) *score = ctx->h_sums[0] / ctx->h_sums[1];
  return MVR_OK;
}

int mvr_apply_pose(mvr_ctx* ctx, const void* points, size_t n, size_t stride_bytes, const double* pose, float* out_xyzw) {
  if (!ctx || !pose || (n && (!points || !out_xyzw))) return MVR_ERR_BAD_ARG;
  if (stride_bytes < 12 || stride_bytes % 4 != 0) return fail(ctx, MVR_ERR_BAD_ARG, "stride must be a multiple of 4 and >= 12");
  if (n > (size_t)INT_MAX / 2) return fail(ctx, MVR_ERR_BAD_ARG, "cloud too large");
  cudaSetDevice(ctx->device);
  if (n == 0) return MVR_OK;
  CK(ctx->scratch.ensure(n * stride_bytes));
  CK(ctx->qtmp.ensure(n * sizeof(float4)));
  CK(cudaMemcpyAsync(ctx->scratch.p, points, n * stride_bytes, cudaMemcpyHostToDevice, ctx->stream));
  CK(launch_apply_pose(ctx->scratch.p, stride_bytes, (int)n, pose, ctx->qtmp.as<float4>(), ctx->stream));
  CK(cudaMemcpyAsync(out_xyzw, ctx->qtmp.p, n * sizeof(float4), cudaMemcpyDeviceToHost, ctx->stream));
  CK(cudaStreamSynchronize(ctx->stream));
  return MVR_OK;
}

int mvr_apply_pose_device(mvr_ctx* ctx, const void* d_points, size_t n, size_t stride_bytes, const double* pose, float* d_out) {
  if (!ctx || !pose || (n && (!d_points || !d_out))) return MVR_ERR_BAD_ARG;
  if (stride_bytes < 12 || stride_bytes % 4 != 0) return fail(ctx, MVR_ERR_BAD_ARG, "stride must be a multiple of 4 and >= 12");
  if (n > (size_t)INT_MAX / 2) return fail(ctx, MVR_ERR_BAD_ARG, "cloud too large");
  cudaSetDevice(ctx->device);
  if (n == 0) return MVR_OK;
  CK(launch_apply_pose(d_points, stride_bytes, (int)n, pose, (float4*)d_out, ctx->stream));
  CK(cudaStreamSynchronize(ctx->stream));
  return MVR_OK;
}

int mvr_merge_registered(mvr_ctx* ctx, const void* const* views, const size_t* counts, const double* poses, const int* registered,
                         int n_views, int full_matrix_normals, void* out, size_t* out_count) {
  if (!ctx || n_views < 0 || !out_count || (n_views && (!views || !counts || !poses))) return MVR_ERR_BAD_ARG;
  cudaSetDevice(ctx->device);
  size_t total = 0;
  for (int v = 0; v < n_views; ++v) {
    if (registered && !registered[v]) continue;
    if (counts[v] && !views[v]) return fail(ctx, MVR_ERR_BAD_ARG, "null view");
    if (counts[v] > (size_t)INT_MAX / 4) return fail(ctx, MVR_ERR_BAD_ARG, "view too large");
    total += counts[v];
  }
  *out_count = total;
  if (!out || total == 0) return MVR_OK;
  CK(ctx->scratch.ensure(total * 48));
  size_t biggest = 0;
  for (int v = 0; v < n_views; ++v) if (!registered || registered[v]) biggest = std::max(biggest, counts[v]);
  CK(ctx->qtmp.ensure(std::max<size_t>(biggest, 1) * 48));
  size_t at = 0;
  for (int v = 0; v < n_views; ++v) {
    if ((registered && !registered[v]) || counts[v] == 0) continue;
    CK(cudaMemcpyAsync(ctx->qtmp.p, views[v], counts[v] * 48, cudaMemcpyHostToDevice, ctx->stream));
    CK(launch_merge_rich(ctx->qtmp.p, (int)counts[v], poses + 16 * v, full_matrix_normals, (char*)ctx->scratch.p + at * 48, ctx->stream));
    at += counts[v];
  }
  CK(cudaMemcpyAsync(out, ctx->scratch.p, total * 48, cudaMemcpyDeviceToHost, ctx->stream));
  CK(cudaStreamSynchronize(ctx->stream));
  return MVR_OK;
}

int mvr_copy_aligned_device(mvr_ctx* ctx, float* d_out) {
  if (!ctx || !d_out) return MVR_ERR_BAD_ARG;
  cudaSetDevice(ctx->device);
  if (!ctx->have_out) return fail(ctx, MVR_ERR_NO_INPUT, "no align has run");
  int rcm = materialize_out(ctx);
  if (rcm) return rcm;
  if (ctx->src.n > 0) CK(cudaMemcpyAsync(d_out, ctx->out_cloud.p, (size_t)ctx->src.n * sizeof(float4), cudaMemcpyDeviceToDevice, ctx->stream));
  CK(cudaStreamSynchronize(ctx->stream));
  return MVR_OK;
}

int mvr_denoise(mvr_ctx* ctx, const void* points, size_t n, size_t stride_bytes, int segment_threshold, double triangle_length,
                int32_t* kept_index, size_t* kept_count, size_t* noise_count) {
  if (!ctx || !kept_count || (n && (!points || !kept_index))) return MVR_ERR_BAD_ARG;
  if (stride_bytes < 12 || stride_bytes % 4 != 0) return fail(ctx, MVR_ERR_BAD_ARG, "stride must be a multiple of 4 and >= 12");
  if (!(triangle_length > 0) || !std::isfinite(triangle_length)) return fail(ctx, MVR_ERR_BAD_ARG, "triangle_length must be positive");
  if (n > (size_t)INT_MAX / 4) return fail(ctx, MVR_ERR_BAD_ARG, "cloud too large");
  cudaSetDevice(ctx->device);
  *kept_count = 0;
  if (noise_count) *noise_count = 0;
  if (n == 0) return MVR_OK;
  const int ni = (int)n;
  CK(ctx->scratch.ensure(n * stride_bytes));
  CK(ctx->qtmp.ensure(n * sizeof(float4)));
  CK(cudaMemcpyAsync(ctx->scratch.p, points, n * stride_bytes, cudaMemcpyHostToDevice, ctx->stream));
  const double I16[16] = {1, 0, 0, 0, 0, 1, 0, 0, 0, 0, 1, 0, 0, 0, 0, 1};
  CK(launch_apply_pose(ctx->scratch.p, stride_bytes, ni, I16, ctx->qtmp.as<float4>(), ctx->stream));
  Cloud tmp;
  tmp.pts = ctx->qtmp.as<float4>(); tmp.n = ni;
  int rc = cloud_bbox(ctx, tmp);
  if (rc) return rc;
  uint32_t cells = 0;
  const PairGrid g = make_pair_grid(tmp.lo, tmp.hi, triangle_length * 1.0001, &cells);
  if ((double)g.cell_lo < triangle_length) return fail(ctx, MVR_ERR_BAD_ARG, "cloud too large for this edge length (grid capped)");
  PairIndex& ix = ctx->nq;
  if ((rc = build_pair_index(ctx, ix, tmp.pts, ni, tmp.n_bad, nullptr, g, cells, false, false))) return rc;
  const size_t nb = (size_t)radix_num_blocks(ni) * 256;
  CK(ctx->itmp.ensure(((size_t)6 * n + nb + 16) * sizeof(uint32_t)));
  uint32_t* parent = ctx->itmp.as<uint32_t>();
  uint32_t *count = parent + n, *keys = count + n, *vals = keys + n, *keys_alt = vals + n, *vals_alt = keys_alt + n, *hist = vals_alt + n, *d_noise = hist + nb;
  CK(cudaMemsetAsync(d_noise, 0, sizeof(uint32_t), ctx->stream));
  CK(launch_denoise_components(ix.sorted.as<float4>(), ix.start.as<uint32_t>(), g, ni, ix.n_valid, triangle_length, parent, keys, count, ctx->stream));
  CK(launch_denoise_keys(count, ni, (uint32_t)std::max(segment_threshold, 0), keys, vals, d_noise, ctx->stream));
  uint32_t *ko = nullptr, *vo = nullptr;
  SortScratch sc{keys_alt, vals_alt, hist};
  CK(launch_radix_sort(keys, vals, ni, 32, sc, &ko, &vo, ctx->stream));
  CK(cudaMemcpyAsync(ctx->h_small, d_noise, sizeof(uint32_t), cudaMemcpyDeviceToHost, ctx->stream));
  CK(cudaStreamSynchronize(ctx->stream));
  const size_t noise = ctx->h_small[0], kept = n - noise;
  if (kept) CK(cudaMemcpyAsync(kept_index, vo, kept * sizeof(uint32_t), cudaMemcpyDeviceToHost, ctx->stream));
  CK(cudaStreamSynchronize(ctx->stream));
  *kept_count = kept;
  if (noise_count) *noise_count = noise;
  ctx->nq.valid = false;
  return MVR_OK;
}

// ... 114 lines not shown
```

### multi-view-registration_b200/csrc/bin.cu

```cuda
#include "launch.h"

namespace mvr {

__global__ void __launch_bounds__(256) k_transform_bin(float4* __restrict__ pts, int n, const float* __restrict__ delta,
                                                       const int* __restrict__ done, GridDev g, uint32_t* __restrict__ keys,
                                                       uint32_t* __restrict__ rank, uint32_t* __restrict__ counters) {
  if (done && *done) return;
  int i = blockIdx.x * blockDim.x + threadIdx.x;
  if (i >= n) return;
  float4 p = pts[i];
  if (delta && finite3(p)) {
    Mat4f M;
#pragma unroll
    for (int k = 0; k < 16; ++k) M.m[k] = __ldg(delta + k);
    p = xform_pinned(M, p);
    pts[i] = p;
  }
  uint32_t key = point_key(p, g);
  keys[i] = key;
  rank[i] = atomicAdd(counters + key, 1u);
}

constexpr int SC_THREADS = 256;
constexpr int SC_ITEMS = 32;
constexpr int SC_TILE = SC_THREADS * SC_ITEMS;

int scan_num_tiles(size_t len) { return (int)((len + SC_TILE - 1) / SC_TILE); }

__device__ __forceinline__ void scan_tiles(uint32_t* __restrict__ counters, uint32_t* __restrict__ start, uint32_t len,
                                           unsigned long long* __restrict__ tile_state, uint32_t epoch, uint32_t ntiles) {
  __shared__ uint32_t warp_sums[SC_THREADS / 32];
  __shared__ uint32_t s_prefix, s_tile;
  if (threadIdx.x == 0) {
    unsigned int* ticket = reinterpret_cast<unsigned int*>(tile_state);
    const unsigned int t = atomicAdd(ticket, 1u);
    if (t == gridDim.x - 1) *ticket = 0u;
    s_tile = t;
  }
  __syncthreads();
  const uint32_t tile = s_tile;
  if (tile >= ntiles) return;
  volatile unsigned long long* st = tile_state + 1;
  const uint32_t base = tile * SC_TILE + threadIdx.x * SC_ITEMS;
  const int lane = threadIdx.x & 31, warp = threadIdx.x >> 5;
  uint32_t v[SC_ITEMS];
  if (base + SC_ITEMS <= len) {
#pragma unroll
    for (int k = 0; k < SC_ITEMS; k += 4) {
      const uint4 a = *reinterpret_cast<const uint4*>(counters + base + k);
      v[k] = a.x; v[k + 1] = a.y; v[k + 2] = a.z; v[k + 3] = a.w;
      *reinterpret_cast<uint4*>(counters + base + k) = make_uint4(0, 0, 0, 0);
    }
  } else {
#pragma unroll
    for (int k = 0; k < SC_ITEMS; ++k) {
      v[k] = (base + k < len) ? counters[base + k] : 0u;
      if (base + k < len) counters[base + k] = 0u;
    }
  }
  uint32_t tsum = 0;
#pragma unroll
  for (int k = 0; k < SC_ITEMS; ++k) tsum += v[k];
  uint32_t incl = tsum;
#pragma unroll
  for (int o = 1; o < 32; o <<= 1) {
    uint32_t t = __shfl_up_sync(0xffffffffu, incl, o);
    if (lane >= o) incl += t;
  }
  if (lane == 31) warp_sums[warp] = incl;
  __syncthreads();
  uint32_t wbase = 0, agg = 0;
#pragma unroll
  for (int w = 0; w < SC_THREADS / 32; ++w) { uint32_t c = warp_sums[w]; if (w < warp) wbase += c; agg += c; }
  const uint32_t texcl = wbase + incl - tsum;

  const unsigned long long tag = (unsigned long long)epoch << 34;
  if (warp == 0) {
    if (tile == 0) {
      if (lane == 0) { st[0] = tag | (2ull << 32) | agg; s_prefix = 0; }
    } else {
      if (lane == 0) st[tile] = tag | (1ull << 32) | agg;
      uint32_t excl = 0;
      int j = (int)tile - 1;
      while (true) {
        const int t = j - lane;
        unsigned long long w = 0;
        bool ready;
        do {
          w = (t >= 0) ? st[t] : (tag | (2ull << 32));
          ready = (w >> 34) == (unsigned long long)epoch && ((w >> 32) & 3ull) != 0;
        } while (!__all_sync(0xffffffffu, ready));
        const uint32_t flag = (uint32_t)(w >> 32) & 3u, val = (uint32_t)w;
        const uint32_t incl_mask = __ballot_sync(0xffffffffu, flag == 2u);
        if (incl_mask) {
          const int first = __ffs(incl_mask) - 1;
          uint32_t c = (lane <= first) ? val : 0u;
#pragma unroll
          for (int o = 16; o > 0; o >>= 1) c += __shfl_xor_sync(0xffffffffu, c, o);
          excl += c;
          break;
        }
        uint32_t c = val;
#pragma unroll
        for (int o = 16; o > 0; o >>= 1) c += __shfl_xor_sync(0xffffffffu, c, o);
        excl += c;
        j -= 32;
      }
      if (lane == 0) { st[tile] = tag | (2ull << 32) | (excl + agg); s_prefix = excl; }
    }
  }
  __syncthreads();
  uint32_t run = s_prefix + texcl;
  if (base + SC_ITEMS <= len) {
#pragma unroll
    for (int k = 0; k < SC_ITEMS; k += 4) {
      uint4 a;
      a.x = run; run += v[k]; a.y = run; run += v[k + 1]; a.z = run; run += v[k + 2]; a.w = run; run += v[k + 3];
      *reinterpret_cast<uint4*>(start + base + k) = a;
    }
  } else {
#pragma unroll
    for (int k = 0; k < SC_ITEMS; ++k) {
      if (base + k < len) start[base + k] = run;
      run += v[k];
    }
  }
  if (tile == ntiles - 1 && threadIdx.x == SC_THREADS - 1) start[len] = s_prefix + agg;
}

__global__ void __launch_bounds__(SC_THREADS) k_scan_cells(uint32_t* __restrict__ counters, uint32_t* __restrict__ start, uint32_t len,
                                                           unsigned long long* __restrict__ tile_state, uint32_t epoch,
                                                           const int* __restrict__ done) {
  if (done && *done) return;
  scan_tiles(counters, start, len, tile_state, epoch, gridDim.x);
}

__global__ void __launch_bounds__(SC_THREADS) k_scan_cells_batch(const __grid_constant__ BuildBatch b) {
  __shared__ uint32_t* s_counters;
  __shared__ uint32_t* s_start;
  __shared__ unsigned long long* s_tiles;
  __shared__ uint32_t s_len, s_epoch, s_ntiles;
  if (threadIdx.x == 0) {
    const BuildJob& j = b.j[blockIdx.y];
    s_counters = j.counters; s_start = j.start; s_tiles = j.tiles; s_len = j.cells + 1u; s_epoch = j.epoch; s_ntiles = (uint32_t)j.ntiles;
  }
  __syncthreads();
  scan_tiles(s_counters, s_start, s_len, s_tiles, s_epoch, s_ntiles);
}

__global__ void __launch_bounds__(256) k_bin_scatter(const float4* __restrict__ pts, int n, const uint32_t* __restrict__ keys,
                                                     const uint32_t* __restrict__ rank, const uint32_t* __restrict__ start,
                                                     const int* __restrict__ done, float4* __restrict__ sorted) {
  if (done && *done) return;
  int i = blockIdx.x * blockDim.x + threadIdx.x;
  if (i >= n) return;
  float4 p = __ldg(pts + i);
  p.w = __int_as_float(i);
  sorted[__ldg(start + __ldg(keys + i)) + __ldg(rank + i)] = p;
}

cudaError_t launch_transform_bin(float4* pts, int n, const float* d_delta, const int* d_done, GridDev g, uint32_t* keys,
                                 uint32_t* rank, uint32_t* counters, cudaStream_t s) {
  if (n <= 0) return cudaSuccess;
  k_transform_bin<<<(n + 255) / 256, 256, 0, s>>>(pts, n, d_delta, d_done, g, keys, rank, counters); count_launch();
  return cudaGetLastError();
}

cudaError_t launch_scan_cells(uint32_t* counters, uint32_t* start, size_t len, unsigned long long* tile_state, uint32_t epoch,
                              const int* d_done, cudaStream_t s) {
  k_scan_cells<<<scan_num_tiles(len), SC_THREADS, 0, s>>>(counters, start, (uint32_t)len, tile_state, epoch, d_done); count_launch();
  return cudaGetLastError();
}

cudaError_t launch_scan_cells_batch(const BuildBatch& batch, int count, int max_tiles, cudaStream_t s) {
  if (count <= 0 || max_tiles <= 0) return cudaSuccess;
  k_scan_cells_batch<<<dim3((unsigned)max_tiles, (unsigned)count), SC_THREADS, 0, s>>>(batch); count_launch();
  return cudaGetLastError();
}

cudaError_t launch_bin_scatter(const float4* pts, int n, const uint32_t* keys, const uint32_t* rank, const uint32_t* start,
                               const int* d_done, float4* sorted, cudaStream_t s) {
  if (n <= 0) return cudaSuccess;
  k_bin_scatter<<<(n + 255) / 256, 256, 0, s>>>(pts, n, keys, rank, start, d_done, sorted); count_launch();
  return cudaGetLastError();
}

}
```

### multi-view-registration_b200/csrc/index.cu

```cuda
#include "launch.h"

namespace mvr {

__host__ __device__ __forceinline__ uint32_t f2ord(float f) {
#ifdef __CUDA_ARCH__
  uint32_t u = __float_as_uint(f);
#else
  uint32_t u; memcpy(&u, &f, 4);
#endif
  return (u & 0x80000000u) ? ~u : (u | 0x80000000u);
}

float bbox_decode(uint32_t e) {
  uint32_t u = (e & 0x80000000u) ? (e & 0x7fffffffu) : ~e;
  float f; memcpy(&f, &u, 4);
  return f;
}

__global__ void k_bbox_init(uint32_t* out) {
  int t = threadIdx.x;
  if (t < 3) out[t] = 0xffffffffu;
  else if (t < 6) out[t] = 0u;
  else if (t == 6) out[t] = 0u;
}
// ... 23 lines not shown
  __shared__ uint32_t s_bad[8];
  const int lane = threadIdx.x & 31, warp = threadIdx.x >> 5;
  if (lane == 0) {
#pragma unroll
    for (int a = 0; a < 3; ++a) { s_lo[warp][a] = lo[a]; s_hi[warp][a] = hi[a]; }
    s_bad[warp] = bad;
  }
  __syncthreads();
  if (threadIdx.x < 3) {
    const int a = threadIdx.x;
    float l = MVR_INF, h = -MVR_INF;
#pragma unroll
    for (int w = 0; w < 8; ++w) { l = fminf(l, s_lo[w][a]); h = fmaxf(h, s_hi[w][a]); }
    if (l <= h) { atomicMin(out + a, f2ord(l)); atomicMax(out + 3 + a, f2ord(h)); }
  } else if (threadIdx.x == 3) {
    uint32_t b = 0;
#pragma unroll
    for (int w = 0; w < 8; ++w) b += s_bad[w];
    if (b) atomicAdd(out + 6, b);
  }
}

__global__ void __launch_bounds__(256) k_bbox(const float4* __restrict__ pts, int n, uint32_t* out) { bbox_body(pts, n, out); }

__global__ void k_bbox_init_batch(uint32_t* out, int count) {
  const int t = blockIdx.x * blockDim.x + threadIdx.x;
  if (t < 7 * count) out[t] = (t % 7 < 3) ? 0xffffffffu : 0u;
}
__global__ void __launch_bounds__(256) k_bbox_batch(const __grid_constant__ BboxBatch b, uint32_t* out) {
  const BboxJob& j = b.j[blockIdx.y];
  bbox_body(j.pts, j.n, out + 7 * blockIdx.y);
}

cudaError_t launch_bbox_init(uint32_t* out7, cudaStream_t s) {
  k_bbox_init<<<1, 32, 0, s>>>(out7); count_launch();
  return cudaGetLastError();
}

cudaError_t launch_bbox_batch(const BboxBatch& batch, int count, uint32_t* out7, cudaStream_t s) {
  if (count <= 0) return cudaSuccess;
  if (count > BBOX_MAX_JOBS) return cudaErrorInvalidValue;
  int max_n = 0;
  for (int k = 0; k < count; ++k) max_n = max(max_n, batch.j[k].n);
  k_bbox_init_batch<<<(7 * count + 255) / 256, 256, 0, s>>>(out7, count); count_launch();
  if (max_n > 0) {
    const int blocks = max(1, min((max_n + 1023) / 1024, (148 * 4 + count - 1) / count));
    k_bbox_batch<<<dim3((unsigned)blocks, (unsigned)count), 256, 0, s>>>(batch, out7); count_launch();
  }
  return cudaGetLastError();
}

cudaError_t launch_bbox(const float4* pts, int n, uint32_t* out7, cudaStream_t s) {
  if (n <= 0) return cudaSuccess;
  int blocks = min((n + 1023) / 1024, 148 * 2);
  k_bbox<<<blocks, 256, 0, s>>>(pts, n, out7); count_launch();
  return cudaGetLastError();
}

__global__ void __launch_bounds__(256) k_morton_keys(const float4* __restrict__ pts, int n, GridDev g,
                                                     uint32_t* __restrict__ keys, uint32_t* __restrict__ vals) {
  int i = blockIdx.x * blockDim.x + threadIdx.x;
  if (i >= n) return;
  keys[i] = point_key(__ldg(pts + i), g);
  vals[i] = (uint32_t)i;
}

__global__ void __launch_bounds__(256) k_transform_keys(float4* __restrict__ pts, int n, Mat4f M, GridDev g,
                                                        uint32_t* __restrict__ keys, uint32_t* __restrict__ vals) {
  int i = blockIdx.x * blockDim.x + threadIdx.x;
  if (i >= n) return;
  float4 p = pts[i];
  if (finite3(p)) { p = xform_pinned(M, p); pts[i] = p; }
  if (keys) { keys[i] = point_key(p, g); vals[i] = (uint32_t)i; }
}

__global__ void __launch_bounds__(256) k_transform(const float4* __restrict__ in, float4* __restrict__ out, int n, Mat4f M) {
  int i = blockIdx.x * blockDim.x + threadIdx.x;
  if (i >= n) return;
  float4 p = __ldg(in + i);
  out[i] = finite3(p) ? xform_pinned(M, p) : p;
}

struct Mat4d { double m[16]; };
__global__ void __launch_bounds__(256) k_apply_pose(const char* __restrict__ in, size_t stride, int n, Mat4d M, float4* __restrict__ out) {
  int i = blockIdx.x * blockDim.x + threadIdx.x;
  if (i >= n) return;
  const float* p = reinterpret_cast<const float*>(in + (size_t)i * stride);
  const double x = p[0], y = p[1], z = p[2];
  float4 r;
  r.x = (float)(M.m[0] * x + M.m[4] * y + M.m[8] * z + M.m[12]);
  r.y = (float)(M.m[1] * x + M.m[5] * y + M.m[9] * z + M.m[13]);
  r.z = (float)(M.m[2] * x + M.m[6] * y + M.m[10] * z + M.m[14]);
  r.w = 1.0f;
  out[i] = r;
}

__global__ void __launch_bounds__(256) k_merge_rich(const float4* __restrict__ in, int n, Mat4d M, int full_matrix_normals, float4* __restrict__ out) {
  const int i = blockIdx.x * blockDim.x + threadIdx.x;
  if (i >= n) return;
  const float4 a = __ldg(in + 3 * (size_t)i), b = __ldg(in + 3 * (size_t)i + 1), c = __ldg(in + 3 * (size_t)i + 2);
  float4 r;
  r.x = (float)(M.m[0] * a.x + M.m[4] * a.y + M.m[8] * a.z + M.m[12]);
  r.y = (float)(M.m[1] * a.x + M.m[5] * a.y + M.m[9] * a.z + M.m[13]);
  r.z = (float)(M.m[2] * a.x + M.m[6] * a.y + M.m[10] * a.z + M.m[14]);
  r.w = a.w;
  const double t = full_matrix_normals ? 1.0 : 0.0;
  float4 q;
  q.x = (float)(M.m[0] * b.x + M.m[4] * b.y + M.m[8] * b.z + t * M.m[12]);
  q.y = (float)(M.m[1] * b.x + M.m[5] * b.y + M.m[9] * b.z + t * M.m[13]);
  q.z = (float)(M.m[2] * b.x + M.m[6] * b.y + M.m[10] * b.z + t * M.m[14]);
  q.w = b.w;
  out[3 * (size_t)i] = r; out[3 * (size_t)i + 1] = q; out[3 * (size_t)i + 2] = c;
}

cudaError_t launch_merge_rich(const void* in48, int n, const double* M16, int full_matrix_normals, void* out48, cudaStream_t s) {
  if (n <= 0) return cudaSuccess;
  Mat4d M;
  for (int k = 0; k < 16; ++k) M.m[k] = M16[k];
  k_merge_rich<<<(n + 255) / 256, 256, 0, s>>>((const float4*)in48, n, M, full_matrix_normals, (float4*)out48); count_launch();
  return cudaGetLastError();
}

cudaError_t launch_apply_pose(const void* in, size_t stride, int n, const double* M16, float4* out, cudaStream_t s) {
  if (n <= 0) return cudaSuccess;
  Mat4d M;
  for (int k = 0; k < 16; ++k) M.m[k] = M16[k];
  k_apply_pose<<<(n + 255) / 256, 256, 0, s>>>((const char*)in, stride, n, M, out); count_launch();
  return cudaGetLastError();
}

cudaError_t launch_morton_keys(const float4* pts, int n, GridDev g, uint32_t* keys, uint32_t* vals, cudaStream_t s) {
  if (n <= 0) return cudaSuccess;
  k_morton_keys<<<(n + 255) / 256, 256, 0, s>>>(pts, n, g, keys, vals); count_launch();
  return cudaGetLastError();
}

cudaError_t launch_transform_keys(float4* pts, int n, Mat4f M, GridDev g, uint32_t* keys, uint32_t* vals, cudaStream_t s) {
  if (n <= 0) return cudaSuccess;
  k_transform_keys<<<(n + 255) / 256, 256, 0, s>>>(pts, n, M, g, keys, vals); count_launch();
  return cudaGetLastError();
}

cudaError_t launch_transform(const float4* in, float4* out, int n, Mat4f M, cudaStream_t s) {
  if (n <= 0) return cudaSuccess;
  k_transform<<<(n + 255) / 256, 256, 0, s>>>(in, out, n, M); count_launch();
  return cudaGetLastError();
}

constexpr int RS_THREADS = 256;
constexpr int RS_WARPS = RS_THREADS / 32;
constexpr int RS_ITEMS = 16;
constexpr int RS_TILE = RS_THREADS * RS_ITEMS;

int radix_num_blocks(int n) { return n > 0 ? (n + RS_TILE - 1) / RS_TILE : 1; }

__global__ void __launch_bounds__(RS_THREADS) k_radix_hist(const uint32_t* __restrict__ keys, int n, int shift,
                                                           uint32_t* __restrict__ hist, int nblk) {
  __shared__ uint32_t h[256];
  h[threadIdx.x] = 0;
  __syncthreads();
  int base = blockIdx.x * RS_TILE;
#pragma unroll 4
  for (int i = threadIdx.x; i < RS_TILE; i += RS_THREADS) {
    int idx = base + i;
    if (idx < n) atomicAdd(&h[(__ldg(keys + idx) >> shift) & 255u], 1u);
  }
  __syncthreads();
  hist[threadIdx.x * nblk + blockIdx.x] = h[threadIdx.x];
}

__global__ void __launch_bounds__(1024) k_radix_scan(uint32_t* __restrict__ hist, int total) {
  __shared__ uint32_t warp_sums[32];
  int per = (total + 1023) / 1024;
  int b = threadIdx.x * per, e = min(b + per, total);
  uint32_t sum = 0;
  for (int i = b; i < e; ++i) sum += hist[i];
  uint32_t incl = sum;
  int lane = threadIdx.x & 31, warp = threadIdx.x >> 5;
#pragma unroll
  for (int o = 1; o < 32; o <<= 1) {
    uint32_t v = __shfl_up_sync(0xffffffffu, incl, o);
    if (lane >= o) incl += v;
  }
  if (lane == 31) warp_sums[warp] = incl;
  __syncthreads();
  if (warp == 0) {
    uint32_t w = warp_sums[lane], wi = w;
#pragma unroll
    for (int o = 1; o < 32; o <<= 1) {
      uint32_t v = __shfl_up_sync(0xffffffffu, wi, o);
      if (lane >= o) wi += v;
    }
    warp_sums[lane] = wi - w;
  }
  __syncthreads();
  uint32_t run = warp_sums[warp] + incl - sum;
  for (int i = b; i < e; ++i) { uint32_t c = hist[i]; hist[i] = run; run += c; }
}

__global__ void __launch_bounds__(RS_THREADS) k_radix_scatter(const uint32_t* __restrict__ kin, const uint32_t* __restrict__ vin,
                                                              uint32_t* __restrict__ kout, uint32_t* __restrict__ vout, int n,
                                                              int shift, const uint32_t* __restrict__ scanned, int nblk) {
  __shared__ uint32_t wc[RS_WARPS][256];
  const int tid = threadIdx.x, warp = tid >> 5, lane = tid & 31;
#pragma unroll
  for (int w = 0; w < RS_WARPS; ++w) wc[w][tid] = 0;
  __syncthreads();
  const int base = blockIdx.x * RS_TILE + warp * (RS_ITEMS * 32);
  uint32_t key[RS_ITEMS];
  uint32_t rank[RS_ITEMS];
#pragma unroll
  for (int r = 0; r < RS_ITEMS; ++r) {
    int idx = base + r * 32 + lane;
    bool valid = idx < n;
    uint32_t live = __ballot_sync(0xffffffffu, valid);
    key[r] = 0; rank[r] = 0;
    if (valid) {
      key[r] = __ldg(kin + idx);
      uint32_t d = (key[r] >> shift) & 255u;
      uint32_t peers = __match_any_sync(live, d);
      int leader = __ffs(peers) - 1;
      uint32_t old = 0;
      if (lane == leader) { old = wc[warp][d]; wc[warp][d] = old + __popc(peers); }
      old = __shfl_sync(peers, old, leader);
      rank[r] = old + __popc(peers & ((1u << lane) - 1u));
    }
    __syncwarp();
  }
  __syncthreads();
  {
    uint32_t run = scanned[tid * nblk + blockIdx.x];
#pragma unroll
    for (int w = 0; w < RS_WARPS; ++w) { uint32_t c = wc[w][tid]; wc[w][tid] = run; run += c; }
  }
  __syncthreads();
#pragma unroll
  for (int r = 0; r < RS_ITEMS; ++r) {
    int idx = base + r * 32 + lane;
    if (idx < n) {
      uint32_t d = (key[r] >> shift) & 255u;
      uint32_t pos = wc[warp][d] + rank[r];
      kout[pos] = key[r];
      vout[pos] = __ldg(vin + idx);
    }
  }
}

cudaError_t launch_radix_sort(uint32_t* keys, uint32_t* vals, int n, int key_bits, SortScratch sc, uint32_t** keys_out,
                              uint32_t** vals_out, cudaStream_t s) {
  *keys_out = keys; *vals_out = vals;
  if (n <= 0) return cudaSuccess;
  int passes = (key_bits + 7) / 8;
  if (passes < 1) passes = 1;
  int nblk = radix_num_blocks(n);
  uint32_t *kin = keys, *vin = vals, *kout = sc.keys_alt, *vout = sc.vals_alt;
  for (int p = 0; p < passes; ++p) {
    int shift = 8 * p;
    k_radix_hist<<<nblk, RS_THREADS, 0, s>>>(kin, n, shift, sc.hist, nblk); count_launch();
    k_radix_scan<<<1, 1024, 0, s>>>(sc.hist, 256 * nblk); count_launch();
    k_radix_scatter<<<nblk, RS_THREADS, 0, s>>>(kin, vin, kout, vout, n, shift, sc.hist, nblk); count_launch();
    uint32_t* t = kin; kin = kout; kout = t;
    t = vin; vin = vout; vout = t;
  }
  *keys_out = kin; *vals_out = vin;
  return cudaGetLastError();
}

__global__ void __launch_bounds__(256) k_gather_sorted(const float4* __restrict__ pts, const uint32_t* __restrict__ perm, int n,
                                                       float4* __restrict__ sorted) {
  int i = blockIdx.x * blockDim.x + threadIdx.x;
  if (i >= n) return;
  uint32_t j = __ldg(perm + i);
  float4 p = __ldg(pts + j);
  p.w = __uint_as_float(j);
  sorted[i] = p;
}

cudaError_t launch_gather_sorted(const float4* pts, const uint32_t* perm, int n, float4* sorted, cudaStream_t s) {
  if (n <= 0) return cudaSuccess;
  k_gather_sorted<<<(n + 255) / 256, 256, 0, s>>>(pts, perm, n, sorted); count_launch();
  return cudaGetLastError();
}

__global__ void __launch_bounds__(256) k_cell_table(const uint32_t* __restrict__ keys, int n, uint32_t C,
                                                    uint32_t* __restrict__ start) {
  long long i = (long long)blockIdx.x * blockDim.x + threadIdx.x;
  const int lane = threadIdx.x & 31;
  long long prev = -1, cur = -1;
  if (i <= n) {
    prev = (i == 0) ? -1 : (long long)min(__ldg(keys + i - 1), C);
    cur = (i < n) ? (long long)min(__ldg(keys + i), C) : (long long)C;
  }
  uint32_t has = __ballot_sync(0xffffffffu, cur > prev);
  while (has) {
    int l = __ffs(has) - 1;
    has &= has - 1;
    long long p = __shfl_sync(0xffffffffu, prev, l), c = __shfl_sync(0xffffffffu, cur, l);
    long long ii = __shfl_sync(0xffffffffu, i, l);
    for (long long k = p + 1 + lane; k <= c; k += 32) start[k] = (uint32_t)ii;
  }
}

cudaError_t launch_cell_table(const uint32_t* sorted_keys, int n, int bits, uint32_t* start, cudaStream_t s) {
  uint32_t C = 1u << (3 * bits);
  long long threads = (long long)n + 1;
  int blocks = (int)((threads + 255) / 256);
  k_cell_table<<<blocks, 256, 0, s>>>(sorted_keys, n, C, start); count_launch();
  return cudaGetLastError();
}

}
```

### multi-view-registration_b200/csrc/launch.h

```cpp
#pragma once
#include <cuda_runtime.h>
#include <stdint.h>

#include "common.cuh"

namespace mvr {

void count_launch(int n = 1);
unsigned long long launch_count();

cudaError_t launch_bbox_init(uint32_t* out7, cudaStream_t s);
cudaError_t launch_bbox(const float4* pts, int n, uint32_t* out7, cudaStream_t s);
float bbox_decode(uint32_t enc);
struct BboxJob { const float4* pts; int n; int pad_; };
enum { BBOX_MAX_JOBS = 64 };
struct BboxBatch { BboxJob j[BBOX_MAX_JOBS]; };
cudaError_t launch_bbox_batch(const BboxBatch& batch, int count, uint32_t* out7, cudaStream_t s);

cudaError_t launch_apply_pose(const void* in, size_t stride, int n, const double* M16, float4* out, cudaStream_t s);

cudaError_t launch_morton_keys(const float4* pts, int n, GridDev g, uint32_t* keys, uint32_t* vals, cudaStream_t s);
cudaError_t launch_transform_keys(float4* pts, int n, Mat4f M, GridDev g, uint32_t* keys, uint32_t* vals, cudaStream_t s);
cudaError_t launch_transform(const float4* in, float4* out, int n, Mat4f M, cudaStream_t s);

struct SortScratch {
  uint32_t* keys_alt;
  uint32_t* vals_alt;
  uint32_t* hist;
};
int radix_num_blocks(int n);
cudaError_t launch_radix_sort(uint32_t* keys, uint32_t* vals, int n, int key_bits, SortScratch sc, uint32_t** keys_out,
                              uint32_t** vals_out, cudaStream_t s);

cudaError_t launch_gather_sorted(const float4* pts, const uint32_t* perm, int n, float4* sorted, cudaStream_t s);
cudaError_t launch_cell_table(const uint32_t* sorted_keys, int n, int bits, uint32_t* start, cudaStream_t s);

cudaError_t launch_transform_bin(float4* pts, int n, const float* d_delta, const int* d_done, GridDev g, uint32_t* keys,
                                 uint32_t* rank, uint32_t* counters, cudaStream_t s);
int scan_num_tiles(size_t len);
cudaError_t launch_scan_cells(uint32_t* counters, uint32_t* start, size_t len, unsigned long long* tile_state, uint32_t epoch,
                              const int* d_done, cudaStream_t s);
cudaError_t launch_bin_scatter(const float4* pts, int n, const uint32_t* keys, const uint32_t* rank, const uint32_t* start,
                               const int* d_done, float4* sorted, cudaStream_t s);

enum { REDUCE_P2P_VALS = 18, REDUCE_P2L_VALS = 30, REDUCE_MOM_VALS = 30, REDUCE_MAX_VALS = 32, REDUCE_BLOCKS = 592, ICP_MAX_LOG = 1024 };

struct IterRec {
  int iteration;
  int n_corr;
  double mse;
  float delta[16];
};

struct IcpState {
  float delta[16];
  double fin[16];
  double sums[REDUCE_MAX_VALS];
  double prev_mse, cur_mse;
  double rot_thr, trans_thr, fit_eps;
  double ox, oy, oz;
  unsigned long long queries;
  int iter, done, reason, status, n_corr;
  int max_iter, fixed, min_corr, p2l, recip, n_src;
  unsigned int ticket;
  long long dbg[8];
  double cum[16];
  double cinv[12];
  float stretch;
  float dev;
  unsigned int n_gate;
  double devd;
  double box[6];
  double babs[3];
};

#ifndef MVR_FUSED_THREADS
#define MVR_FUSED_THREADS 256
#endif
enum { FUSED_THREADS = MVR_FUSED_THREADS, FUSED_WARPS = FUSED_THREADS / 32, FUSED_MAX_BLOCKS = 148 * 8 * (256 / FUSED_THREADS) };

struct BuildJob {
  const float4* in;
  int n, apply;
  Mat4f M;
  PairGrid g;
  uint32_t cells;
  uint32_t* keys;
  uint32_t* rank;
  uint32_t* counters;
  unsigned long long* tiles;
  uint32_t epoch;
  int ntiles;
  float4* tmp;
  float4* sorted;
  uint32_t* start;
  uint32_t* crowded;
  int ordered;
  int pad_;
};
enum { BUILD_MAX_JOBS = 48 };
struct BuildBatch { BuildJob j[BUILD_MAX_JOBS]; };
cudaError_t launch_pair_builds(const BuildBatch& batch, int count, cudaStream_t s);
cudaError_t launch_scan_cells_batch(const BuildBatch& batch, int count, int max_tiles, cudaStream_t s);
cudaError_t launch_gate_mask(const uint32_t* start, PairGrid g, int wstride, int D, int Dx, uint32_t* occ, uint32_t* mask, cudaStream_t s);
struct FwdArgs {
  float4* cur;
  int n_valid;
  const float4* tgt;
  const uint32_t* tstart;
  PairGrid gt;
  int m_valid;
  int32_t* corr_p;
  uint32_t* rmin;
  double max2;
  float max_d2f;
  const uint32_t* gmask;
  int gm_stride;
  const float4* nrm;
  double* partials;
  IcpState* st;
  IterRec* log;
  int grid;
  float4* nsrc;
};
struct RevArgs {
  const float4* tgt;
  int m_valid;
  uint32_t* rmin;
  const float4* cur;
  const uint32_t* sstart;
  PairGrid gs;
  int n_valid;
  const int32_t* corr_p;
  int32_t* rnn;
  const float4* nrm;
  double* partials;
  IcpState* st;
  IterRec* log;
  int grid;
  int per;
  const float4* nsrc;
};
enum { EST_P2P = 0, EST_P2L = 1, EST_MOM = 2 , EST_SYM = 3  };
enum { FUSED_MAX_PAIRS = 24 };
struct FwdBatch { FwdArgs a[FUSED_MAX_PAIRS]; };
struct RevBatch { RevArgs a[FUSED_MAX_PAIRS]; };
static_assert(sizeof(FwdBatch) + sizeof(int) <= 32764 && sizeof(RevBatch) <= 32764, "a group's arguments must fit the kernel parameters");
struct InitJob {
  int32_t* corr_p; int n; int m; uint32_t* rmin; IcpState* st; uint32_t* crowded;
  float4* nsrc; const float4* snrm; const float4* sorted; int n_valid; int pad_;
  Mat4f M;
};
struct InitBatch { InitJob j[BUILD_MAX_JOBS]; };
static_assert(sizeof(InitBatch) + sizeof(void*) <= 32764, "the batch's jobs must fit the kernel parameters");
cudaError_t launch_align_init(const InitBatch& batch, int count, const IcpState* stage, cudaStream_t s);
cudaError_t launch_align_gather(const InitBatch& batch, int count, IcpState* stage, cudaStream_t s);
int fused_grid(int items);
int fused_grid_rev(int items);
int fused_rev_chunks(int items);
cudaError_t launch_icp_forward(const FwdBatch& batch, int pairs, int max_grid, int first, bool reciprocal, int est, cudaStream_t s);
cudaError_t launch_icp_reverse(const RevBatch& batch, int pairs, int max_grid, int est, cudaStream_t s);
cudaError_t launch_pair_nn(const float4* q, int n, bool by_w, const float4* tgt_sorted, const uint32_t* tstart, PairGrid g, int m_valid,
                           int32_t* out_idx, float* out_d2, cudaStream_t s);
cudaError_t launch_resolve_pairs(const float4* src_sorted, int n_valid, const int32_t* corr_p, const int32_t* rnn, const float4* tgt_sorted,
                                 int32_t* corr_j, float* corr_d2, cudaStream_t s);
cudaError_t launch_transform_final(const float4* in, float4* out, int n, const IcpState* st, cudaStream_t s);
cudaError_t launch_reduce_fitness(const int32_t* idx, const float* d2, int n, double max_range, double* partials,
                                  double* out, cudaStream_t s);

size_t compact_scratch_elems(int n);
cudaError_t launch_compact_corr(const int32_t* corr_j, const float* corr_d2, int n, uint32_t* scratch, int32_t* out_q,
                                int32_t* out_m, float* out_d2, uint32_t* count_out, cudaStream_t s);

cudaError_t launch_merge_rich(const void* in48, int n, const double* M16, int full_matrix_normals, void* out48, cudaStream_t s);

cudaError_t launch_cell_nn(const float4* q_sorted, int nq, const uint32_t* d_nq_valid, const float4* tgt_sorted, const uint32_t* tstart,
                           PairGrid g, int m_valid, int32_t* out_idx, float* out_d2, cudaStream_t s);

cudaError_t launch_seeded_nn(const float4* q_sorted, int nq, const uint32_t* d_nq_valid, const float4* tgt_sorted, const uint32_t* tstart,
                             PairGrid g, int m_valid, int32_t* out_idx, float* out_d2, cudaStream_t s);

cudaError_t launch_warp_nn(const float4* q, int n, const float4* tgt_sorted, const uint32_t* tstart, PairGrid g, int m_valid, int32_t* out_idx,
                           float* out_d2, cudaStream_t s);

cudaError_t launch_denoise_components(const float4* sorted, const uint32_t* start, PairGrid g, int n, int n_valid, double threshold,
                                      uint32_t* parent, uint32_t* root, uint32_t* count, cudaStream_t s);
cudaError_t launch_denoise_keys(const uint32_t* count, int n, uint32_t segment_threshold, uint32_t* keys, uint32_t* vals,
                                uint32_t* n_noise, cudaStream_t s);

struct NormalsJob {
  const float4* sorted;
  const uint32_t* start;
  PairGrid g;
  int n, n_valid;
  float3 viewpoint;
  float4* out;
  int32_t* nbr;
};
struct NormalsBatch { NormalsJob j[BUILD_MAX_JOBS]; };
cudaError_t launch_normals(const NormalsBatch& batch, int count, int k, cudaStream_t s);

}
```

### multi-view-registration_b200/csrc/pair_index.cu

```cuda
#include <algorithm>

#include "launch.h"
#include "pair_search.cuh"

namespace mvr {

__device__ __forceinline__ const BuildJob& load_job(const BuildBatch& b, BuildJob& s_job) {
  static_assert(sizeof(BuildJob) % 4 == 0 && sizeof(BuildJob) / 4 <= 256, "job block");
  if (threadIdx.x < sizeof(BuildJob) / 4) ((uint32_t*)&s_job)[threadIdx.x] = ((const uint32_t*)&b.j[blockIdx.y])[threadIdx.x];
  __syncthreads();
  return s_job;
}

__global__ void __launch_bounds__(256) k_pair_count(const __grid_constant__ BuildBatch b) {
  __shared__ BuildJob s_job;
  const BuildJob& j = load_job(b, s_job);
  const int i = blockIdx.x * blockDim.x + threadIdx.x;
  if (i >= j.n) return;
  float4 p = __ldg(j.in + i);
  const bool ok = finite3(p);
  if (j.apply && ok) p = xform_pinned(j.M, p);
  const uint32_t key = ok ? pg_key(p, j.g) : j.cells;
  j.keys[i] = key;
  j.rank[i] = atomicAdd(j.counters + key, 1u);
}

__global__ void __launch_bounds__(256) k_pair_scatter(const __grid_constant__ BuildBatch b) {
  __shared__ BuildJob s_job;
  const BuildJob& j = load_job(b, s_job);
  const int i = blockIdx.x * blockDim.x + threadIdx.x;
  if (i >= j.n) return;
  float4 p = __ldg(j.in + i);
  if (j.apply && finite3(p)) p = xform_pinned(j.M, p);
  p.w = __uint_as_float((uint32_t)i);
  (j.ordered ? j.tmp : j.sorted)[__ldg(j.start + __ldg(j.keys + i)) + __ldg(j.rank + i)] = p;
}

constexpr uint32_t RERANK_LIMIT = 1024;
__global__ void __launch_bounds__(256) k_pair_rerank(const __grid_constant__ BuildBatch b) {
  __shared__ BuildJob s_job;
  const BuildJob& j = load_job(b, s_job);
  const int k = blockIdx.x * blockDim.x + threadIdx.x;
  if (k >= j.n || !j.ordered) return;
  const float4* __restrict__ tmp = j.tmp;
  const float4 p = __ldg(tmp + k);
  const uint32_t idx = __float_as_uint(p.w);
  const uint32_t key = __ldg(j.keys + idx);
  const uint32_t s = __ldg(j.start + key), e = __ldg(j.start + key + 1);
  if (e - s > RERANK_LIMIT) {
    j.sorted[k] = p;
    if (j.crowded && (uint32_t)k == s) atomicMax(j.crowded, e - s);
    return;
  }
  uint32_t r = 0;
  for (uint32_t q = s; q < e; ++q) r += (__float_as_uint(__ldg(&tmp[q].w)) < idx) ? 1u : 0u;
  j.sorted[s + r] = p;
}

__global__ void __launch_bounds__(256) k_gate_occ(const uint32_t* __restrict__ start, PairGrid g, int wstride, size_t words, uint32_t* __restrict__ occ) {
  const size_t w = (size_t)blockIdx.x * blockDim.x + threadIdx.x;
  if (w >= words) return;
  const size_t row = w / (size_t)wstride;
  const int xw = (int)(w % (size_t)wstride);
  const uint32_t* r = start + row * (size_t)g.nx;
  uint32_t bits = 0;
  uint32_t prev = __ldg(r + xw * 32);
  for (int b = 0; b < 32; ++b) {
    const int x = xw * 32 + b;
    if (x >= g.nx) break;
    const uint32_t next = __ldg(r + x + 1);
    if (next > prev) bits |= 1u << b;
    prev = next;
  }
  occ[w] = bits;
}

__global__ void __launch_bounds__(256) k_gate_dilate(const uint32_t* __restrict__ occ, PairGrid g, int wstride, int D, int Dx, size_t words, uint32_t* __restrict__ out) {
  const size_t w = (size_t)blockIdx.x * blockDim.x + threadIdx.x;
  if (w >= words) return;
  const int xw = (int)(w % (size_t)wstride);
  const size_t row = w / (size_t)wstride;
  const int y = (int)(row % (size_t)g.ny), z = (int)(row / (size_t)g.ny);
  uint32_t acc = 0;
  for (int zz = max(z - D, 0); zz <= min(z + D, g.nz - 1); ++zz)
    for (int yy = max(y - D, 0); yy <= min(y + D, g.ny - 1); ++yy) {
      const uint32_t* r = occ + ((size_t)zz * g.ny + yy) * wstride;
      const uint32_t cur = __ldg(r + xw), prev = xw > 0 ? __ldg(r + xw - 1) : 0u, next = xw + 1 < wstride ? __ldg(r + xw + 1) : 0u;
      uint32_t v = cur;
      for (int k = 1; k <= Dx; ++k) v |= (cur << k) | (cur >> k) | (prev >> (32 - k)) | (next << (32 - k));
      acc |= v;
    }
  out[w] = acc;
}

cudaError_t launch_gate_mask(const uint32_t* start, PairGrid g, int wstride, int D, int Dx, uint32_t* occ, uint32_t* mask, cudaStream_t s) {
  const size_t words = (size_t)g.ny * g.nz * wstride;
  if (words == 0 || D < 1 || Dx < 1 || Dx > 31) return cudaErrorInvalidValue;
  const unsigned blocks = (unsigned)((words + 255) / 256);
  k_gate_occ<<<blocks, 256, 0, s>>>(start, g, wstride, words, occ); count_launch();
  k_gate_dilate<<<blocks, 256, 0, s>>>(occ, g, wstride, D, Dx, words, mask); count_launch();
  return cudaGetLastError();
}

cudaError_t launch_pair_builds(const BuildBatch& batch, int count, cudaStream_t s) {
  if (count <= 0) return cudaSuccess;
  if (count > BUILD_MAX_JOBS) return cudaErrorInvalidValue;
  int max_n = 0, max_tiles = 0;
  bool any_ordered = false;
  for (int k = 0; k < count; ++k) {
    max_n = std::max(max_n, batch.j[k].n);
    max_tiles = std::max(max_tiles, batch.j[k].ntiles);
    any_ordered = any_ordered || batch.j[k].ordered;
  }
  const dim3 gp((unsigned)std::max((max_n + 255) / 256, 1), (unsigned)count);
  if (max_n > 0) { k_pair_count<<<gp, 256, 0, s>>>(batch); count_launch(); }
  launch_scan_cells_batch(batch, count, max_tiles, s);
  if (max_n > 0) { k_pair_scatter<<<gp, 256, 0, s>>>(batch); count_launch(); }
  if (max_n > 0 && any_ordered) { k_pair_rerank<<<gp, 256, 0, s>>>(batch); count_launch(); }
  return cudaGetLastError();
}

}
```

Baseline: 14.77 billion.

## Replace atomic counting-sort pair index build with batched LSD radix sort

```diff
diff --git a/include/mvr_b200.h b/include/mvr_b200.h
--- a/include/mvr_b200.h
+++ b/include/mvr_b200.h
@@ -92,6 +92,7 @@
 int mvr_ctx_set_profiling(mvr_ctx* ctx, int on);
 int mvr_ctx_get_kernel_stats(mvr_ctx* ctx, mvr_kernel_stat* out , int reset);
 double mvr_debug_value(mvr_ctx* ctx, int k);
+int mvr_debug_pair_index(mvr_ctx* ctx, int which, size_t* n, uint32_t* cells, double* grid, float* sorted, uint32_t* start);
 int mvr_ctx_set_index_options(mvr_ctx* ctx, float cell_edge, int max_bits);
 
 int mvr_ctx_set_nn_options(mvr_ctx* ctx, double points_per_cell, double dense_ratio);
diff --git a/multi-view-registration_b200/__init__.py b/multi-view-registration_b200/__init__.py
--- a/multi-view-registration_b200/__init__.py
+++ b/multi-view-registration_b200/__init__.py
@@ -170,6 +170,7 @@
     L.mvr_ctx_get_kernel_stats.argtypes = [vp, C.POINTER(KernelStat), C.c_int]
     L.mvr_debug_value.argtypes = [vp, C.c_int]
     L.mvr_debug_value.restype = C.c_double
+    L.mvr_debug_pair_index.argtypes = [vp, C.c_int, C.POINTER(C.c_size_t), C.POINTER(C.c_uint32), C.POINTER(C.c_double), fp, up]
     L.mvr_ctx_set_index_options.argtypes = [vp, C.c_float, C.c_int]
     L.mvr_ctx_set_batch_group.argtypes = [vp, C.c_int]
     L.mvr_ctx_set_nn_options.argtypes = [vp, C.c_double, C.c_double]
@@ -349,6 +350,17 @@
     def debug_value(self, k):
         return float(lib().mvr_debug_value(self._h, int(k)))
 
+    def debug_pair_index(self, which):
+        n, cells = C.c_size_t(0), C.c_uint32(0)
+        g = np.zeros(8, dtype=np.float64)
+        self._ck(lib().mvr_debug_pair_index(self._h, int(which), C.byref(n), C.byref(cells), _dp(g), None, None))
+        sorted_ = np.empty((n.value, 4), dtype=np.float32)
+        start = np.empty(cells.value + 2, dtype=np.uint32)
+        self._ck(lib().mvr_debug_pair_index(self._h, int(which), C.byref(n), C.byref(cells), None, _fp(sorted_), _up(start)))
+        grid = dict(origin=g[:3].astype(np.float32), inv_cell_x=np.float32(g[3]), inv_cell=np.float32(g[4]),
+                    n=tuple(int(v) for v in g[5:]), cells=int(cells.value))
+        return sorted_, start, grid
+
     def set_index_options(self, cell_edge=0.0, max_bits=8):
         self._ck(lib().mvr_ctx_set_index_options(self._h, C.c_float(cell_edge), int(max_bits)))
 
diff --git a/multi-view-registration_b200/build.py b/multi-view-registration_b200/build.py
--- a/multi-view-registration_b200/build.py
+++ b/multi-view-registration_b200/build.py
@@ -8,7 +8,7 @@
 HOST = os.path.join(HERE, "host")
 LIB = os.path.join(HERE, "libmvr_b200.so")
 
-CU_SOURCES = ["index.cu", "bin.cu", "pair_index.cu", "cell_nn.cu", "icp.cu", "normals.cu", "denoise.cu", "api.cu"]
+CU_SOURCES = ["index.cu", "pair_index.cu", "cell_nn.cu", "icp.cu", "normals.cu", "denoise.cu", "api.cu"]
 HOST_SOURCES = ["registrator.cpp", "lum.cpp", "capi.cpp", "multi.cpp"]
 
 NVCC_FLAGS = [
diff --git a/multi-view-registration_b200/csrc/api.cu b/multi-view-registration_b200/csrc/api.cu
--- a/multi-view-registration_b200/csrc/api.cu
+++ b/multi-view-registration_b200/csrc/api.cu
@@ -82,7 +82,7 @@
   int gm_stride = 0;
   PairGrid g{};
   uint32_t cells = 0;
-  int n_valid = 0;
+  int n = 0, n_valid = 0;
   uint64_t gen = 0;
   bool valid = false;
   void release() { sorted.release(); start.release(); s0.release(); gocc.release(); gmask.release(); gm_gate = -1.f; valid = false; }
@@ -111,7 +111,7 @@
   FwdArgs fa{}; RevArgs ra{};
   bool want_rnn = false;
   int group_pairs = 0;
-  struct BuildScratch { DevBuf keys, vals, moved, count, tiles; uint32_t epoch = 1; } bs[2];
+  struct BuildScratch { DevBuf keys, vals, keys_alt, vals_alt, hist; } bs[2];
   DevBuf stage_dev;
   IcpState* h_stage = nullptr;
   int stage_cap = 0;
@@ -301,9 +301,9 @@
 PairGrid make_pair_grid(const float lo[3], const float hi[3], double e, uint32_t* cells_out, int xr = 1);
 bool same_pair_grid(const PairGrid& a, const PairGrid& b);
 int build_pair_index(mvr_ctx* ctx, PairIndex& ix, const float4* pts, int n, int n_bad, const Mat4f* guess, const PairGrid& g,
-                     uint32_t cells, bool keep_s0, bool ordered = true);
+                     uint32_t cells, bool keep_s0, bool report = true);
 int plan_pair_index(mvr_ctx* ctx, PairIndex& ix, int slot, const float4* pts, int n, int n_bad, const Mat4f* guess, const PairGrid& g,
-                    uint32_t cells, bool ordered, cudaStream_t stream, BuildJob* job);
+                    uint32_t cells, bool report, cudaStream_t stream, BuildJob* job);
 int run_pair_builds(mvr_ctx* ctx, const BuildJob* jobs, int count, cudaStream_t stream);
 
 double pair_cell_edge(mvr_ctx* ctx, const Cloud& c, double max_dist);
@@ -410,36 +410,28 @@
 bool same_pair_grid(const PairGrid& a, const PairGrid& b) { return std::memcmp(&a, &b, sizeof(PairGrid)) == 0; }
 
 int plan_pair_index(mvr_ctx* ctx, PairIndex& ix, int slot, const float4* pts, int n, int n_bad, const Mat4f* guess, const PairGrid& g,
-                    uint32_t cells, bool ordered, cudaStream_t stream, BuildJob* job) {
+                    uint32_t cells, bool report, cudaStream_t stream, BuildJob* job) {
   mvr_ctx::BuildScratch& bs = ctx->bs[slot];
   const size_t nn = (size_t)std::max(n, 1);
   CK(bs.keys.ensure(nn * sizeof(uint32_t)));
   CK(bs.vals.ensure(nn * sizeof(uint32_t)));
-  if (ordered) CK(bs.moved.ensure(nn * sizeof(float4)));
+  CK(bs.keys_alt.ensure(nn * sizeof(uint32_t)));
+  CK(bs.vals_alt.ensure(nn * sizeof(uint32_t)));
+  CK(bs.hist.ensure((size_t)256 * radix_num_blocks(n) * sizeof(uint32_t)));
   CK(ix.sorted.ensure(nn * sizeof(float4)));
   CK(ix.start.ensure(((size_t)cells + 2) * sizeof(uint32_t)));
-  if (((size_t)cells + 1) * sizeof(uint32_t) > bs.count.cap) {
-    CK(bs.count.ensure(((size_t)cells + 1) * sizeof(uint32_t)));
-    CK(cudaMemsetAsync(bs.count.p, 0, bs.count.cap, stream));
-  }
-  const int ntiles = scan_num_tiles((size_t)cells + 1);
-  const size_t tiles = (size_t)ntiles + 1;
-  if (tiles * sizeof(unsigned long long) > bs.tiles.cap) {
-    CK(bs.tiles.ensure(tiles * sizeof(unsigned long long)));
-    CK(cudaMemsetAsync(bs.tiles.p, 0, bs.tiles.cap, stream));
-  }
   if (!ctx->crowded.p) { CK(ctx->crowded.ensure(64)); CK(cudaMemsetAsync(ctx->crowded.p, 0, 64, stream)); }
   BuildJob& j = *job;
   j = BuildJob{};
   j.in = pts; j.n = n; j.apply = guess ? 1 : 0;
   if (guess) j.M = *guess;
   j.g = g; j.cells = cells;
-  j.keys = bs.keys.as<uint32_t>(); j.rank = bs.vals.as<uint32_t>(); j.counters = bs.count.as<uint32_t>();
-  j.tiles = bs.tiles.as<unsigned long long>(); j.epoch = bs.epoch; j.ntiles = ntiles;
-  bs.epoch = (bs.epoch % 0x3fffffffu) + 1;
-  j.tmp = ordered ? bs.moved.as<float4>() : nullptr; j.sorted = ix.sorted.as<float4>(); j.start = ix.start.as<uint32_t>();
-  j.crowded = ctx->crowded.as<uint32_t>(); j.ordered = ordered ? 1 : 0;
-  ix.g = g; ix.cells = cells; ix.n_valid = n - n_bad; ix.valid = true; ix.gm_gate = -1.f;
+  j.keys[0] = bs.keys.as<uint32_t>(); j.keys[1] = bs.keys_alt.as<uint32_t>();
+  j.vals[0] = bs.vals.as<uint32_t>(); j.vals[1] = bs.vals_alt.as<uint32_t>();
+  j.hist = bs.hist.as<uint32_t>();
+  j.sorted = ix.sorted.as<float4>(); j.start = ix.start.as<uint32_t>();
+  j.crowded = report ? ctx->crowded.as<uint32_t>() : nullptr;
+  ix.g = g; ix.cells = cells; ix.n = n; ix.n_valid = n - n_bad; ix.valid = true; ix.gm_gate = -1.f;
   return MVR_OK;
 }
 
@@ -447,8 +439,11 @@
   for (int k0 = 0; k0 < count; k0 += BUILD_MAX_JOBS) {
     const int c = std::min(count - k0, (int)BUILD_MAX_JOBS);
     BuildBatch batch;
+    uint32_t max_cells = 0;
+    for (int k = 0; k < c; ++k) max_cells = std::max(max_cells, jobs[k0 + k].cells);
+    const double per_point = 64.0 + 20.0 * radix_passes(max_cells);
     double bytes = 0, pts = 0;
-    for (int k = 0; k < c; ++k) { batch.j[k] = jobs[k0 + k]; bytes += 32.0 * jobs[k0 + k].n + 8.0 * jobs[k0 + k].cells; pts += jobs[k0 + k].n; }
+    for (int k = 0; k < c; ++k) { batch.j[k] = jobs[k0 + k]; bytes += per_point * jobs[k0 + k].n + 4.0 * (jobs[k0 + k].cells + 2.0); pts += jobs[k0 + k].n; }
     ProfScope ps(ctx, MVR_K_SORT, bytes, pts, 1, stream);
     CK(launch_pair_builds(batch, c, stream));
   }
@@ -456,11 +451,11 @@
 }
 
 int build_pair_index(mvr_ctx* ctx, PairIndex& ix, const float4* pts, int n, int n_bad, const Mat4f* guess, const PairGrid& g,
-                     uint32_t cells, bool keep_s0, bool ordered) {
+                     uint32_t cells, bool keep_s0, bool report) {
   (void)keep_s0;
   BuildJob job;
   ix.valid = false;
-  int rc = plan_pair_index(ctx, ix, &ix == &ctx->pt || &ix == &ctx->nt ? 0 : 1, pts, n, n_bad, guess, g, cells, ordered, ctx->stream, &job);
+  int rc = plan_pair_index(ctx, ix, &ix == &ctx->pt || &ix == &ctx->nt ? 0 : 1, pts, n, n_bad, guess, g, cells, report, ctx->stream, &job);
   if (rc) { ix.valid = false; return rc; }
   return run_pair_builds(ctx, &job, 1, ctx->stream);
 }
@@ -586,7 +581,7 @@
   if (ctx->ev_b) cudaEventDestroy(ctx->ev_b);
   ctx->tgt.release(); ctx->src.release(); ctx->normals.release(); ctx->snormals.release(); ctx->nsrc.release();
   ctx->pt.release(); ctx->ps.release(); ctx->nt.release(); ctx->nq.release();
-  for (auto& b : ctx->bs) { b.keys.release(); b.vals.release(); b.moved.release(); b.count.release(); b.tiles.release(); }
+  for (auto& b : ctx->bs) { b.keys.release(); b.vals.release(); b.keys_alt.release(); b.vals_alt.release(); b.hist.release(); }
   ctx->stage_dev.release(); ctx->bbox_dev.release();
   if (ctx->h_stage) cudaFreeHost(ctx->h_stage);
   if (ctx->h_bbox) cudaFreeHost(ctx->h_bbox);
@@ -1257,7 +1252,7 @@
     report->gpu_ms = (double)ms / (double)std::max(batch_pairs, 1);
   }
   if (ctx->crowded_seen)
-    ctx->err = "warning: a grid cell holds " + std::to_string(ctx->crowded_seen) + " points (duplicates or clamped outliers?): index build and search slow down, sums over it lose their fixed order";
+    ctx->err = "warning: a grid cell holds " + std::to_string(ctx->crowded_seen) + " points (duplicates or clamped outliers?): searches through it slow down";
   if (h.status == MVR_ERR_TOO_FEW_CORRESPONDENCES) ctx->err = "not enough correspondences";
   if (h.status == MVR_ERR_NOT_SPD) ctx->err = h.p2l == 2 ? "symmetric point-to-plane normal equations not positive definite" : "point-to-plane normal equations not positive definite";
   return h.status;
@@ -1394,6 +1389,22 @@
   if (ctx && k == 8) return (double)ctx->crowded_seen;
   if (!ctx || !ctx->h_state || k < 0 || k >= 8) return 0.0;
   return (double)ctx->h_state->dbg[k];
+}
+
+int mvr_debug_pair_index(mvr_ctx* ctx, int which, size_t* n, uint32_t* cells, double* grid, float* sorted, uint32_t* start) {
+  if (!ctx || !n || !cells || (which != MVR_CLOUD_TARGET && which != MVR_CLOUD_SOURCE)) return MVR_ERR_BAD_ARG;
+  cudaSetDevice(ctx->device);
+  const PairIndex& ix = which == MVR_CLOUD_TARGET ? ctx->pt : ctx->ps;
+  if (!ix.valid) return fail(ctx, MVR_ERR_NO_INPUT, "no per-align index (run an align first)");
+  *n = (size_t)ix.n; *cells = ix.cells;
+  if (grid) {
+    const double g[8] = {ix.g.ox, ix.g.oy, ix.g.oz, ix.g.inv_cell_x, ix.g.inv_cell, (double)ix.g.nx, (double)ix.g.ny, (double)ix.g.nz};
+    std::memcpy(grid, g, sizeof(g));
+  }
+  if (sorted && ix.n) CK(cudaMemcpyAsync(sorted, ix.sorted.p, (size_t)ix.n * sizeof(float4), cudaMemcpyDeviceToHost, ctx->stream));
+  if (start) CK(cudaMemcpyAsync(start, ix.start.p, ((size_t)ix.cells + 2) * sizeof(uint32_t), cudaMemcpyDeviceToHost, ctx->stream));
+  CK(cudaStreamSynchronize(ctx->stream));
+  return MVR_OK;
 }
 
 int mvr_icp_get_iterations(mvr_ctx* ctx, mvr_icp_iteration* out, int max_records, int* count) {
diff --git a/multi-view-registration_b200/csrc/bin.cu b/multi-view-registration_b200/csrc/bin.cu
--- a/multi-view-registration_b200/csrc/bin.cu
+++ /dev/null
@@ -1,188 +0,0 @@
-#include "launch.h"
-
-namespace mvr {
-
-__global__ void __launch_bounds__(256) k_transform_bin(float4* __restrict__ pts, int n, const float* __restrict__ delta,
-                                                       const int* __restrict__ done, GridDev g, uint32_t* __restrict__ keys,
-                                                       uint32_t* __restrict__ rank, uint32_t* __restrict__ counters) {
-  if (done && *done) return;
-  int i = blockIdx.x * blockDim.x + threadIdx.x;
-  if (i >= n) return;
-  float4 p = pts[i];
-  if (delta && finite3(p)) {
-    Mat4f M;
-#pragma unroll
-    for (int k = 0; k < 16; ++k) M.m[k] = __ldg(delta + k);
-    p = xform_pinned(M, p);
-    pts[i] = p;
-  }
-  uint32_t key = point_key(p, g);
-  keys[i] = key;
-  rank[i] = atomicAdd(counters + key, 1u);
-}
-
-constexpr int SC_THREADS = 256;
-constexpr int SC_ITEMS = 32;
-constexpr int SC_TILE = SC_THREADS * SC_ITEMS;
-
-int scan_num_tiles(size_t len) { return (int)((len + SC_TILE - 1) / SC_TILE); }
-
-__device__ __forceinline__ void scan_tiles(uint32_t* __restrict__ counters, uint32_t* __restrict__ start, uint32_t len,
-                                           unsigned long long* __restrict__ tile_state, uint32_t epoch, uint32_t ntiles) {
-  __shared__ uint32_t warp_sums[SC_THREADS / 32];
-  __shared__ uint32_t s_prefix, s_tile;
-  if (threadIdx.x == 0) {
-    unsigned int* ticket = reinterpret_cast<unsigned int*>(tile_state);
-    const unsigned int t = atomicAdd(ticket, 1u);
-    if (t == gridDim.x - 1) *ticket = 0u;
-    s_tile = t;
-  }
-  __syncthreads();
-  const uint32_t tile = s_tile;
-  if (tile >= ntiles) return;
-  volatile unsigned long long* st = tile_state + 1;
-  const uint32_t base = tile * SC_TILE + threadIdx.x * SC_ITEMS;
-  const int lane = threadIdx.x & 31, warp = threadIdx.x >> 5;
-  uint32_t v[SC_ITEMS];
-  if (base + SC_ITEMS <= len) {
-#pragma unroll
-    for (int k = 0; k < SC_ITEMS; k += 4) {
-      const uint4 a = *reinterpret_cast<const uint4*>(counters + base + k);
-      v[k] = a.x; v[k + 1] = a.y; v[k + 2] = a.z; v[k + 3] = a.w;
-      *reinterpret_cast<uint4*>(counters + base + k) = make_uint4(0, 0, 0, 0);
-    }
-  } else {
-#pragma unroll
-    for (int k = 0; k < SC_ITEMS; ++k) {
-      v[k] = (base + k < len) ? counters[base + k] : 0u;
-      if (base + k < len) counters[base + k] = 0u;
-    }
-  }
-  uint32_t tsum = 0;
-#pragma unroll
-  for (int k = 0; k < SC_ITEMS; ++k) tsum += v[k];
-  uint32_t incl = tsum;
-#pragma unroll
-  for (int o = 1; o < 32; o <<= 1) {
-    uint32_t t = __shfl_up_sync(0xffffffffu, incl, o);
-    if (lane >= o) incl += t;
-  }
-  if (lane == 31) warp_sums[warp] = incl;
-  __syncthreads();
-  uint32_t wbase = 0, agg = 0;
-#pragma unroll
-  for (int w = 0; w < SC_THREADS / 32; ++w) { uint32_t c = warp_sums[w]; if (w < warp) wbase += c; agg += c; }
-  const uint32_t texcl = wbase + incl - tsum;
-
-  const unsigned long long tag = (unsigned long long)epoch << 34;
-  if (warp == 0) {
-    if (tile == 0) {
-      if (lane == 0) { st[0] = tag | (2ull << 32) | agg; s_prefix = 0; }
-    } else {
-      if (lane == 0) st[tile] = tag | (1ull << 32) | agg;
-      uint32_t excl = 0;
-      int j = (int)tile - 1;
-      while (true) {
-        const int t = j - lane;
-        unsigned long long w = 0;
-        bool ready;
-        do {
-          w = (t >= 0) ? st[t] : (tag | (2ull << 32));
-          ready = (w >> 34) == (unsigned long long)epoch && ((w >> 32) & 3ull) != 0;
-        } while (!__all_sync(0xffffffffu, ready));
-        const uint32_t flag = (uint32_t)(w >> 32) & 3u, val = (uint32_t)w;
-        const uint32_t incl_mask = __ballot_sync(0xffffffffu, flag == 2u);
-        if (incl_mask) {
-          const int first = __ffs(incl_mask) - 1;
-          uint32_t c = (lane <= first) ? val : 0u;
-#pragma unroll
-          for (int o = 16; o > 0; o >>= 1) c += __shfl_xor_sync(0xffffffffu, c, o);
-          excl += c;
-          break;
-        }
-        uint32_t c = val;
-#pragma unroll
-        for (int o = 16; o > 0; o >>= 1) c += __shfl_xor_sync(0xffffffffu, c, o);
-        excl += c;
-        j -= 32;
-      }
-      if (lane == 0) { st[tile] = tag | (2ull << 32) | (excl + agg); s_prefix = excl; }
-    }
-  }
-  __syncthreads();
-  uint32_t run = s_prefix + texcl;
-  if (base + SC_ITEMS <= len) {
-#pragma unroll
-    for (int k = 0; k < SC_ITEMS; k += 4) {
-      uint4 a;
-      a.x = run; run += v[k]; a.y = run; run += v[k + 1]; a.z = run; run += v[k + 2]; a.w = run; run += v[k + 3];
-      *reinterpret_cast<uint4*>(start + base + k) = a;
-    }
-  } else {
-#pragma unroll
-    for (int k = 0; k < SC_ITEMS; ++k) {
-      if (base + k < len) start[base + k] = run;
-      run += v[k];
-    }
-  }
-  if (tile == ntiles - 1 && threadIdx.x == SC_THREADS - 1) start[len] = s_prefix + agg;
-}
-
-__global__ void __launch_bounds__(SC_THREADS) k_scan_cells(uint32_t* __restrict__ counters, uint32_t* __restrict__ start, uint32_t len,
-                                                           unsigned long long* __restrict__ tile_state, uint32_t epoch,
-                                                           const int* __restrict__ done) {
-  if (done && *done) return;
-  scan_tiles(counters, start, len, tile_state, epoch, gridDim.x);
-}
-
-__global__ void __launch_bounds__(SC_THREADS) k_scan_cells_batch(const __grid_constant__ BuildBatch b) {
-  __shared__ uint32_t* s_counters;
-  __shared__ uint32_t* s_start;
-  __shared__ unsigned long long* s_tiles;
-  __shared__ uint32_t s_len, s_epoch, s_ntiles;
-  if (threadIdx.x == 0) {
-    const BuildJob& j = b.j[blockIdx.y];
-    s_counters = j.counters; s_start = j.start; s_tiles = j.tiles; s_len = j.cells + 1u; s_epoch = j.epoch; s_ntiles = (uint32_t)j.ntiles;
-  }
-  __syncthreads();
-  scan_tiles(s_counters, s_start, s_len, s_tiles, s_epoch, s_ntiles);
-}
-
-__global__ void __launch_bounds__(256) k_bin_scatter(const float4* __restrict__ pts, int n, const uint32_t* __restrict__ keys,
-                                                     const uint32_t* __restrict__ rank, const uint32_t* __restrict__ start,
-                                                     const int* __restrict__ done, float4* __restrict__ sorted) {
-  if (done && *done) return;
-  int i = blockIdx.x * blockDim.x + threadIdx.x;
-  if (i >= n) return;
-  float4 p = __ldg(pts + i);
-  p.w = __int_as_float(i);
-  sorted[__ldg(start + __ldg(keys + i)) + __ldg(rank + i)] = p;
-}
-
-cudaError_t launch_transform_bin(float4* pts, int n, const float* d_delta, const int* d_done, GridDev g, uint32_t* keys,
-                                 uint32_t* rank, uint32_t* counters, cudaStream_t s) {
-  if (n <= 0) return cudaSuccess;
-  k_transform_bin<<<(n + 255) / 256, 256, 0, s>>>(pts, n, d_delta, d_done, g, keys, rank, counters); count_launch();
-  return cudaGetLastError();
-}
-
-cudaError_t launch_scan_cells(uint32_t* counters, uint32_t* start, size_t len, unsigned long long* tile_state, uint32_t epoch,
-                              const int* d_done, cudaStream_t s) {
-  k_scan_cells<<<scan_num_tiles(len), SC_THREADS, 0, s>>>(counters, start, (uint32_t)len, tile_state, epoch, d_done); count_launch();
-  return cudaGetLastError();
-}
-
-cudaError_t launch_scan_cells_batch(const BuildBatch& batch, int count, int max_tiles, cudaStream_t s) {
-  if (count <= 0 || max_tiles <= 0) return cudaSuccess;
-  k_scan_cells_batch<<<dim3((unsigned)max_tiles, (unsigned)count), SC_THREADS, 0, s>>>(batch); count_launch();
-  return cudaGetLastError();
-}
-
-cudaError_t launch_bin_scatter(const float4* pts, int n, const uint32_t* keys, const uint32_t* rank, const uint32_t* start,
-                               const int* d_done, float4* sorted, cudaStream_t s) {
-  if (n <= 0) return cudaSuccess;
-  k_bin_scatter<<<(n + 255) / 256, 256, 0, s>>>(pts, n, keys, rank, start, d_done, sorted); count_launch();
-  return cudaGetLastError();
-}
-
-}
diff --git a/multi-view-registration_b200/csrc/index.cu b/multi-view-registration_b200/csrc/index.cu
--- a/multi-view-registration_b200/csrc/index.cu
+++ b/multi-view-registration_b200/csrc/index.cu
@@ -199,24 +199,30 @@
 constexpr int RS_ITEMS = 16;
 constexpr int RS_TILE = RS_THREADS * RS_ITEMS;
 
-int radix_num_blocks(int n) { return n > 0 ? (n + RS_TILE - 1) / RS_TILE : 1; }
-
-__global__ void __launch_bounds__(RS_THREADS) k_radix_hist(const uint32_t* __restrict__ keys, int n, int shift,
-                                                           uint32_t* __restrict__ hist, int nblk) {
+__host__ __device__ __forceinline__ int rs_blocks(int n) { return n > 0 ? (n + RS_TILE - 1) / RS_TILE : 1; }
+int radix_num_blocks(int n) { return rs_blocks(n); }
+int radix_passes(uint32_t max_key) {
+  int bits = 0;
+  while (bits < 32 && (max_key >> bits) != 0u) ++bits;
+  return bits > 0 ? (bits + 7) / 8 : 1;
+}
+
+__device__ __forceinline__ void radix_hist_body(const uint32_t* __restrict__ keys, int n, int shift, uint32_t* __restrict__ hist,
+                                                int nblk, int blk) {
   __shared__ uint32_t h[256];
   h[threadIdx.x] = 0;
   __syncthreads();
-  int base = blockIdx.x * RS_TILE;
+  int base = blk * RS_TILE;
 #pragma unroll 4
   for (int i = threadIdx.x; i < RS_TILE; i += RS_THREADS) {
     int idx = base + i;
     if (idx < n) atomicAdd(&h[(__ldg(keys + idx) >> shift) & 255u], 1u);
   }
   __syncthreads();
-  hist[threadIdx.x * nblk + blockIdx.x] = h[threadIdx.x];
-}
-
-__global__ void __launch_bounds__(1024) k_radix_scan(uint32_t* __restrict__ hist, int total) {
+  hist[threadIdx.x * nblk + blk] = h[threadIdx.x];
+}
+
+__device__ __forceinline__ void radix_scan_body(uint32_t* __restrict__ hist, int total) {
   __shared__ uint32_t warp_sums[32];
   int per = (total + 1023) / 1024;
   int b = threadIdx.x * per, e = min(b + per, total);
@@ -245,15 +251,15 @@
   for (int i = b; i < e; ++i) { uint32_t c = hist[i]; hist[i] = run; run += c; }
 }
 
-__global__ void __launch_bounds__(RS_THREADS) k_radix_scatter(const uint32_t* __restrict__ kin, const uint32_t* __restrict__ vin,
-                                                              uint32_t* __restrict__ kout, uint32_t* __restrict__ vout, int n,
-                                                              int shift, const uint32_t* __restrict__ scanned, int nblk) {
+__device__ __forceinline__ void radix_scatter_body(const uint32_t* __restrict__ kin, const uint32_t* __restrict__ vin,
+                                                   uint32_t* __restrict__ kout, uint32_t* __restrict__ vout, int n, int shift,
+                                                   const uint32_t* __restrict__ scanned, int nblk, int blk) {
   __shared__ uint32_t wc[RS_WARPS][256];
   const int tid = threadIdx.x, warp = tid >> 5, lane = tid & 31;
 #pragma unroll
   for (int w = 0; w < RS_WARPS; ++w) wc[w][tid] = 0;
   __syncthreads();
-  const int base = blockIdx.x * RS_TILE + warp * (RS_ITEMS * 32);
+  const int base = blk * RS_TILE + warp * (RS_ITEMS * 32);
   uint32_t key[RS_ITEMS];
   uint32_t rank[RS_ITEMS];
 #pragma unroll
@@ -276,7 +282,7 @@
   }
   __syncthreads();
   {
-    uint32_t run = scanned[tid * nblk + blockIdx.x];
+    uint32_t run = scanned[tid * nblk + blk];
 #pragma unroll
     for (int w = 0; w < RS_WARPS; ++w) { uint32_t c = wc[w][tid]; wc[w][tid] = run; run += c; }
   }
@@ -291,6 +297,38 @@
       vout[pos] = __ldg(vin + idx);
     }
   }
+}
+
+__global__ void __launch_bounds__(RS_THREADS) k_radix_hist(const uint32_t* __restrict__ keys, int n, int shift,
+                                                           uint32_t* __restrict__ hist, int nblk) {
+  radix_hist_body(keys, n, shift, hist, nblk, blockIdx.x);
+}
+
+__global__ void __launch_bounds__(1024) k_radix_scan(uint32_t* __restrict__ hist, int total) { radix_scan_body(hist, total); }
+
+__global__ void __launch_bounds__(RS_THREADS) k_radix_scatter(const uint32_t* __restrict__ kin, const uint32_t* __restrict__ vin,
+                                                              uint32_t* __restrict__ kout, uint32_t* __restrict__ vout, int n,
+                                                              int shift, const uint32_t* __restrict__ scanned, int nblk) {
+  radix_scatter_body(kin, vin, kout, vout, n, shift, scanned, nblk, blockIdx.x);
+}
+
+__global__ void __launch_bounds__(RS_THREADS) k_pair_sort_hist(const __grid_constant__ BuildBatch b, int shift, int src) {
+  const BuildJob& j = b.j[blockIdx.y];
+  const int nblk = rs_blocks(j.n);
+  if ((int)blockIdx.x >= nblk) return;
+  radix_hist_body(j.keys[src], j.n, shift, j.hist, nblk, blockIdx.x);
+}
+
+__global__ void __launch_bounds__(1024) k_pair_sort_scan(const __grid_constant__ BuildBatch b) {
+  const BuildJob& j = b.j[blockIdx.x];
+  radix_scan_body(j.hist, 256 * rs_blocks(j.n));
+}
+
+__global__ void __launch_bounds__(RS_THREADS) k_pair_sort_scatter(const __grid_constant__ BuildBatch b, int shift, int src) {
+  const BuildJob& j = b.j[blockIdx.y];
+  const int nblk = rs_blocks(j.n);
+  if ((int)blockIdx.x >= nblk) return;
+  radix_scatter_body(j.keys[src], j.vals[src], j.keys[src ^ 1], j.vals[src ^ 1], j.n, shift, j.hist, nblk, blockIdx.x);
 }
 
 cudaError_t launch_radix_sort(uint32_t* keys, uint32_t* vals, int n, int key_bits, SortScratch sc, uint32_t** keys_out,
@@ -313,6 +351,20 @@
   return cudaGetLastError();
 }
 
+cudaError_t launch_radix_sort_batch(const BuildBatch& batch, int count, int passes, cudaStream_t s) {
+  if (count <= 0) return cudaSuccess;
+  if (count > BUILD_MAX_JOBS) return cudaErrorInvalidValue;
+  int max_blk = 1;
+  for (int k = 0; k < count; ++k) max_blk = max(max_blk, radix_num_blocks(batch.j[k].n));
+  const dim3 grid((unsigned)max_blk, (unsigned)count);
+  for (int p = 0; p < passes; ++p) {
+    k_pair_sort_hist<<<grid, RS_THREADS, 0, s>>>(batch, 8 * p, p & 1); count_launch();
+    k_pair_sort_scan<<<count, 1024, 0, s>>>(batch); count_launch();
+    k_pair_sort_scatter<<<grid, RS_THREADS, 0, s>>>(batch, 8 * p, p & 1); count_launch();
+  }
+  return cudaGetLastError();
+}
+
 __global__ void __launch_bounds__(256) k_gather_sorted(const float4* __restrict__ pts, const uint32_t* __restrict__ perm, int n,
                                                        float4* __restrict__ sorted) {
   int i = blockIdx.x * blockDim.x + threadIdx.x;
diff --git a/multi-view-registration_b200/csrc/launch.h b/multi-view-registration_b200/csrc/launch.h
--- a/multi-view-registration_b200/csrc/launch.h
+++ b/multi-view-registration_b200/csrc/launch.h
@@ -34,14 +34,6 @@
 
 cudaError_t launch_gather_sorted(const float4* pts, const uint32_t* perm, int n, float4* sorted, cudaStream_t s);
 cudaError_t launch_cell_table(const uint32_t* sorted_keys, int n, int bits, uint32_t* start, cudaStream_t s);
-
-cudaError_t launch_transform_bin(float4* pts, int n, const float* d_delta, const int* d_done, GridDev g, uint32_t* keys,
-                                 uint32_t* rank, uint32_t* counters, cudaStream_t s);
-int scan_num_tiles(size_t len);
-cudaError_t launch_scan_cells(uint32_t* counters, uint32_t* start, size_t len, unsigned long long* tile_state, uint32_t epoch,
-                              const int* d_done, cudaStream_t s);
-cudaError_t launch_bin_scatter(const float4* pts, int n, const uint32_t* keys, const uint32_t* rank, const uint32_t* start,
-                               const int* d_done, float4* sorted, cudaStream_t s);
 
 enum { REDUCE_P2P_VALS = 18, REDUCE_P2L_VALS = 30, REDUCE_MOM_VALS = 30, REDUCE_MAX_VALS = 32, REDUCE_BLOCKS = 592, ICP_MAX_LOG = 1024 };
 
@@ -85,23 +77,19 @@
   Mat4f M;
   PairGrid g;
   uint32_t cells;
-  uint32_t* keys;
-  uint32_t* rank;
-  uint32_t* counters;
-  unsigned long long* tiles;
-  uint32_t epoch;
-  int ntiles;
-  float4* tmp;
+  int pad_;
+  uint32_t* keys[2];
+  uint32_t* vals[2];
+  uint32_t* hist;
   float4* sorted;
   uint32_t* start;
   uint32_t* crowded;
-  int ordered;
-  int pad_;
 };
-enum { BUILD_MAX_JOBS = 48 };
+enum { BUILD_MAX_JOBS = 48, CROWDED_CELL = 1024 };
 struct BuildBatch { BuildJob j[BUILD_MAX_JOBS]; };
 cudaError_t launch_pair_builds(const BuildBatch& batch, int count, cudaStream_t s);
-cudaError_t launch_scan_cells_batch(const BuildBatch& batch, int count, int max_tiles, cudaStream_t s);
+int radix_passes(uint32_t max_key);
+cudaError_t launch_radix_sort_batch(const BuildBatch& batch, int count, int passes, cudaStream_t s);
 cudaError_t launch_gate_mask(const uint32_t* start, PairGrid g, int wstride, int D, int Dx, uint32_t* occ, uint32_t* mask, cudaStream_t s);
 struct FwdArgs {
   float4* cur;
diff --git a/multi-view-registration_b200/csrc/pair_index.cu b/multi-view-registration_b200/csrc/pair_index.cu
--- a/multi-view-registration_b200/csrc/pair_index.cu
+++ b/multi-view-registration_b200/csrc/pair_index.cu
@@ -12,7 +12,7 @@
   return s_job;
 }
 
-__global__ void __launch_bounds__(256) k_pair_count(const __grid_constant__ BuildBatch b) {
+__global__ void __launch_bounds__(256) k_pair_keys(const __grid_constant__ BuildBatch b) {
   __shared__ BuildJob s_job;
   const BuildJob& j = load_job(b, s_job);
   const int i = blockIdx.x * blockDim.x + threadIdx.x;
@@ -20,41 +20,91 @@
   float4 p = __ldg(j.in + i);
   const bool ok = finite3(p);
   if (j.apply && ok) p = xform_pinned(j.M, p);
-  const uint32_t key = ok ? pg_key(p, j.g) : j.cells;
-  j.keys[i] = key;
-  j.rank[i] = atomicAdd(j.counters + key, 1u);
+  j.keys[0][i] = ok ? pg_key(p, j.g) : j.cells;
+  j.vals[0][i] = (uint32_t)i;
 }
 
-__global__ void __launch_bounds__(256) k_pair_scatter(const __grid_constant__ BuildBatch b) {
-  __shared__ BuildJob s_job;
-  const BuildJob& j = load_job(b, s_job);
-  const int i = blockIdx.x * blockDim.x + threadIdx.x;
-  if (i >= j.n) return;
-  float4 p = __ldg(j.in + i);
-  if (j.apply && finite3(p)) p = xform_pinned(j.M, p);
-  p.w = __uint_as_float((uint32_t)i);
-  (j.ordered ? j.tmp : j.sorted)[__ldg(j.start + __ldg(j.keys + i)) + __ldg(j.rank + i)] = p;
+constexpr int FILL_THREADS = 256;
+__device__ __forceinline__ void block_lower_bound2(const uint32_t* __restrict__ keys, uint32_t n, uint32_t v0, uint32_t v1,
+                                                   uint32_t& r0, uint32_t& r1) {
+  uint32_t lo0 = 0, hi0 = n, lo1 = 0, hi1 = n;
+  while (hi0 > lo0 || hi1 > lo1) {
+    const uint32_t st0 = (hi0 - lo0 + FILL_THREADS - 1) / FILL_THREADS, st1 = (hi1 - lo1 + FILL_THREADS - 1) / FILL_THREADS;
+    const uint32_t p0 = lo0 + threadIdx.x * st0, p1 = lo1 + threadIdx.x * st1;
+    const bool b0 = p0 < hi0 && __ldg(keys + p0) < v0;
+    const bool b1 = p1 < hi1 && __ldg(keys + p1) < v1;
+    const uint32_t c0 = (uint32_t)__syncthreads_count(b0), c1 = (uint32_t)__syncthreads_count(b1);
+    if (c0 == 0) hi0 = lo0; else { hi0 = min(lo0 + c0 * st0, hi0); lo0 += (c0 - 1) * st0 + 1; }
+    if (c1 == 0) hi1 = lo1; else { hi1 = min(lo1 + c1 * st1, hi1); lo1 += (c1 - 1) * st1 + 1; }
+  }
+  r0 = lo0; r1 = lo1;
 }
 
-constexpr uint32_t RERANK_LIMIT = 1024;
-__global__ void __launch_bounds__(256) k_pair_rerank(const __grid_constant__ BuildBatch b) {
+constexpr int FILL_PER = 32;
+constexpr int FILL_TILE = FILL_THREADS * FILL_PER;
+__global__ void __launch_bounds__(FILL_THREADS) k_pair_fill(const __grid_constant__ BuildBatch b, int src) {
   __shared__ BuildJob s_job;
+  __shared__ uint32_t s_first[FILL_THREADS * (FILL_PER + 1)];
+  __shared__ uint32_t s_after[FILL_THREADS];
+  __shared__ uint32_t s_warp[FILL_THREADS / 32];
   const BuildJob& j = load_job(b, s_job);
-  const int k = blockIdx.x * blockDim.x + threadIdx.x;
-  if (k >= j.n || !j.ordered) return;
-  const float4* __restrict__ tmp = j.tmp;
-  const float4 p = __ldg(tmp + k);
-  const uint32_t idx = __float_as_uint(p.w);
-  const uint32_t key = __ldg(j.keys + idx);
-  const uint32_t s = __ldg(j.start + key), e = __ldg(j.start + key + 1);
-  if (e - s > RERANK_LIMIT) {
+  const uint32_t n = (uint32_t)j.n;
+  const uint32_t* __restrict__ keys = j.keys[src];
+  const uint32_t* __restrict__ vals = j.vals[src];
+  for (uint32_t k = blockIdx.x * FILL_THREADS + threadIdx.x; k < n; k += gridDim.x * FILL_THREADS) {
+    const uint32_t idx = __ldg(vals + k);
+    float4 p = __ldg(j.in + idx);
+    if (j.apply && finite3(p)) p = xform_pinned(j.M, p);
+    p.w = __uint_as_float(idx);
     j.sorted[k] = p;
-    if (j.crowded && (uint32_t)k == s) atomicMax(j.crowded, e - s);
+  }
+  const uint32_t len = j.cells + 2u;
+  const uint32_t c0 = blockIdx.x * FILL_TILE;
+  if (c0 >= len) return;
+  uint32_t lo, hi;
+  block_lower_bound2(keys, n, c0, c0 + FILL_TILE, lo, hi);
+  const uint32_t tend = min(len - c0, (uint32_t)FILL_TILE);
+  if (lo == hi) {
+    for (uint32_t c = threadIdx.x; c < tend; c += FILL_THREADS) j.start[c0 + c] = lo;
     return;
   }
-  uint32_t r = 0;
-  for (uint32_t q = s; q < e; ++q) r += (__float_as_uint(__ldg(&tmp[q].w)) < idx) ? 1u : 0u;
-  j.sorted[s + r] = p;
+  const int t = threadIdx.x, lane = t & 31, warp = t >> 5;
+  uint32_t* mine = s_first + t * (FILL_PER + 1);
+#pragma unroll
+  for (int i = 0; i < FILL_PER; ++i) mine[i] = 0xffffffffu;
+  __syncthreads();
+  for (uint32_t k = lo + t; k < hi; k += FILL_THREADS) {
+    const uint32_t key = __ldg(keys + k);
+    if (k == lo || __ldg(keys + k - 1) != key) {
+      const uint32_t c = key - c0;
+      s_first[(c / FILL_PER) * (FILL_PER + 1) + c % FILL_PER] = k;
+    }
+  }
+  __syncthreads();
+  uint32_t run = 0xffffffffu;
+#pragma unroll
+  for (int i = FILL_PER - 1; i >= 0; --i) { run = min(run, mine[i]); mine[i] = run; }
+  uint32_t incl = run;
+#pragma unroll
+  for (int o = 1; o < 32; o <<= 1) {
+    const uint32_t v = __shfl_down_sync(0xffffffffu, incl, o);
+    if (lane + o < 32) incl = min(incl, v);
+  }
+  if (lane == 0) s_warp[warp] = incl;
+  uint32_t next = __shfl_down_sync(0xffffffffu, incl, 1);
+  if (lane == 31) next = 0xffffffffu;
+  __syncthreads();
+  uint32_t after = hi;
+  for (int w = warp + 1; w < FILL_THREADS / 32; ++w) after = min(after, s_warp[w]);
+  s_after[t] = min(after, next);
+  __syncthreads();
+  for (uint32_t c = t; c < tend; c += FILL_THREADS) {
+    const uint32_t s = min(s_first[(c / FILL_PER) * (FILL_PER + 1) + c % FILL_PER], s_after[c / FILL_PER]);
+    j.start[c0 + c] = s;
+    const uint32_t c1 = c + 1;
+    const uint32_t e = c1 < FILL_TILE ? min(s_first[(c1 / FILL_PER) * (FILL_PER + 1) + c1 % FILL_PER], s_after[c1 / FILL_PER]) : hi;
+    if (j.crowded && c0 + c <= j.cells && e - s > CROWDED_CELL) atomicMax(j.crowded, e - s);
+  }
 }
 
 __global__ void __launch_bounds__(256) k_gate_occ(const uint32_t* __restrict__ start, PairGrid g, int wstride, size_t words, uint32_t* __restrict__ occ) {
@@ -105,18 +155,23 @@
 cudaError_t launch_pair_builds(const BuildBatch& batch, int count, cudaStream_t s) {
   if (count <= 0) return cudaSuccess;
   if (count > BUILD_MAX_JOBS) return cudaErrorInvalidValue;
-  int max_n = 0, max_tiles = 0;
-  bool any_ordered = false;
+  int max_n = 0;
+  uint32_t max_cells = 0, max_len = 0;
   for (int k = 0; k < count; ++k) {
     max_n = std::max(max_n, batch.j[k].n);
-    max_tiles = std::max(max_tiles, batch.j[k].ntiles);
-    any_ordered = any_ordered || batch.j[k].ordered;
+    max_cells = std::max(max_cells, batch.j[k].cells);
+    max_len = std::max(max_len, batch.j[k].cells + 2u);
   }
-  const dim3 gp((unsigned)std::max((max_n + 255) / 256, 1), (unsigned)count);
-  if (max_n > 0) { k_pair_count<<<gp, 256, 0, s>>>(batch); count_launch(); }
-  launch_scan_cells_batch(batch, count, max_tiles, s);
-  if (max_n > 0) { k_pair_scatter<<<gp, 256, 0, s>>>(batch); count_launch(); }
-  if (max_n > 0 && any_ordered) { k_pair_rerank<<<gp, 256, 0, s>>>(batch); count_launch(); }
+  int src = 0;
+  if (max_n > 0) {
+    k_pair_keys<<<dim3((unsigned)((max_n + 255) / 256), (unsigned)count), 256, 0, s>>>(batch); count_launch();
+    const int passes = radix_passes(max_cells);
+    cudaError_t e = launch_radix_sort_batch(batch, count, passes, s);
+    if (e != cudaSuccess) return e;
+    src = passes & 1;
+  }
+  const unsigned fx = std::max((max_len + FILL_TILE - 1) / FILL_TILE, (unsigned)((max_n + 1023) / 1024));
+  k_pair_fill<<<dim3(fx, (unsigned)count), FILL_THREADS, 0, s>>>(batch, src); count_launch();
   return cudaGetLastError();
 }
 
```

New measurement: 13.82 billion (median of 6 runs). 0.936x the previous value.
